# yynil/RWKV_LM_EXT

Hardware: AMD Instinct MI355X
Metric: WKV6 fwd+bwd tokens/sec/GPU (B=8,T=4096,C=2048) + %HBM roofline (higher is better)
Workload: dtype bf16

## Files before the change

### rwkv_lm_ext_amd/_build.py

```python
import os
import shutil
import subprocess

PKG_DIR = os.path.dirname(os.path.abspath(__file__))
CSRC = os.path.join(PKG_DIR, "csrc")
LIB_PATH = os.path.join(PKG_DIR, "librwkv6_amd.so")
SOURCES = ["wkv6_scan.hip", "wkv5_scan.hip", "wkv6_chunk.hip", "wkv6_chunk_bwd12k.hip", "wkv6_mix.hip", "wkv6_lora.hip", "wkv6_api.hip"]
HEADERS = ["wkv6_common.h", "wkv6_scan.h", "wkv5_scan.h", "wkv6_chunk.h", os.path.join("..", "..", "include", "wkv6_amd.h")]
HIPCC_FLAGS = ["--offload-arch=gfx950", "-O3", "-std=c++17", "-fPIC", "-fno-strict-aliasing", "-Wall", "-Wno-unused-function"]


def _hipcc():
    return shutil.which("hipcc") or "/opt/rocm/bin/hipcc"


def needs_build():
    if not os.path.exists(LIB_PATH):
        return True
    t = os.path.getmtime(LIB_PATH)
    deps = [os.path.join(CSRC, s) for s in SOURCES + HEADERS] + [os.path.abspath(__file__)]
    return any(os.path.exists(d) and os.path.getmtime(d) > t for d in deps)


def build(force=False, verbose=False):
    import fcntl
    import tempfile
    if not force and not needs_build():
        return LIB_PATH
    with open(LIB_PATH + ".lock", "w") as lock:
        fcntl.flock(lock, fcntl.LOCK_EX)
        try:
            if not force and not needs_build():
                return LIB_PATH
            with tempfile.TemporaryDirectory(prefix="rwkv6_build_", dir=PKG_DIR) as tmp:
                objs = []
                for src in SOURCES:
                    obj = os.path.join(tmp, src.replace(".hip", ".o"))
                    cmd = [_hipcc()] + HIPCC_FLAGS + ["-c", os.path.join(CSRC, src), "-o", obj]
                    if verbose:
                        print(" ".join(cmd))
                    subprocess.check_call(cmd)
                    objs.append(obj)
                out = os.path.join(tmp, "librwkv6_amd.so")
                cmd = [_hipcc(), "--offload-arch=gfx950", "-shared", "-fPIC", "-o", out] + objs
                if verbose:
                    print(" ".join(cmd))
                subprocess.check_call(cmd)
                os.replace(out, LIB_PATH)
            return LIB_PATH
        finally:
            fcntl.flock(lock, fcntl.LOCK_UN)


if __name__ == "__main__":
    print(build(force=True, verbose=True))
```

### rwkv_lm_ext_amd/csrc/wkv6_chunk_bwd12k.hip

```cpp
#include <type_traits>
#include "wkv6_chunk.h"

namespace wkv6 {

namespace {

using namespace chunk;

enum { R_RH = 0, R_RL, R_GY, R_R, R_K, NR_ARR };
enum { K_KH = 0, K_KL, K_V, NK_ARR };
constexpr int FRS = 72 * 4;
constexpr int ROFF_FR = NR_ARR * ARR;
constexpr int ROFF_LW = ROFF_FR + BLK * FRS;
constexpr int ROFF_E8 = ROFF_LW + BLK * FRS;
constexpr int ROFF_COEF = ROFF_E8 + 256;
constexpr int ROFF_VG = ROFF_COEF + 128;
constexpr int RBLK_BYTES = ROFF_VG + 128;
constexpr int KOFF_E16 = NK_ARR * ARR;
constexpr int KOFF_E16M8 = KOFF_E16 + 256;
constexpr int KBLK_BYTES = KOFF_E16M8 + 256;
constexpr int STG = 32, SBLK = STG / BLK;
constexpr int RBUF_BYTES = SBLK * RBLK_BYTES;
constexpr int KBUF_BYTES = SBLK * KBLK_BYTES;
constexpr int KRING = 3;
constexpr int KP_OFF = 2 * RBUF_BYTES;
constexpr int CKT = CKPT_TOK;
constexpr int XT_OFF = KP_OFF + KRING * KBUF_BYTES;
constexpr int XS_OFF = XT_OFF + 4 * 1024;
constexpr int XFLAG_OFF = 128;
constexpr int GRS = 144;
constexpr int GOP_OFF = XS_OFF + 2 * 1024;
constexpr int TAG_DA = 0, TAG_SC = 4, TAG_GA = 8, TAG_GB = 12, TAG_GC = 16, TAG_GD = 20, N_TAGS = 24;
constexpr int BWD12K_LDS = GOP_OFF + 2 * HEAD * GRS;
static_assert(BWD12K_LDS <= 160 * 1024, "LDS budget");

#define WKV6_DPP_ACC4(x, ctrl) asm("s_nop 1\n\t" \
    "v_add_f32_dpp %0, %0, %0 " ctrl " row_mask:0xf bank_mask:0xf\n\t" "v_add_f32_dpp %1, %1, %1 " ctrl " row_mask:0xf bank_mask:0xf\n\t" \
    "v_add_f32_dpp %2, %2, %2 " ctrl " row_mask:0xf bank_mask:0xf\n\t" "v_add_f32_dpp %3, %3, %3 " ctrl " row_mask:0xf bank_mask:0xf" \
    : "+v"(x[0]), "+v"(x[1]), "+v"(x[2]), "+v"(x[3]))

__device__ __forceinline__ void split8(const float (&t0)[4], const float (&t1)[4], b8v& hi, b8v& lo, const SplitConst& spc)
{
    uint2 h0, l0, h1, l1;
    split4(t0, h0, l0, spc);
    split4(t1, h1, l1, spc);
    hi = __builtin_bit_cast(b8v, make_uint4(h0.x, h0.y, h1.x, h1.y));
    lo = __builtin_bit_cast(b8v, make_uint4(l0.x, l0.y, l1.x, l1.y));
}

enum : unsigned {
    BWD_W_RAW = 1u << 0,
    BWD_SPLIT = 1u << 1,
    BWD_AFF = 1u << 2,
    BWD_CLK = 1u << 3,
    BWD_CHAIN = 1u << 4,
    BWD_VARLEN = 1u << 5,
};
constexpr unsigned bit(bool on, unsigned b) { return on ? b : 0u; }
struct BwdChain {
    int b, ntok;
    int ko, ro;
    bool chained_in;
    bool nx_chain;
    unsigned nx_bh;
    int nx_b, nx_ntok;
    bool nx_rev, nx_use_u;
    const float* nx_ckpt;
};
struct BwdCarry {
    uint2 pr[2], pk[2], pw[2];
    float4 pe[2];
    uint2 ck_[2];
    float cfr[2][4], clw[2][4], cc8[4];
    uint2 cvp[2];
    f4v CK[4];
};
template <unsigned MODE, int GEN = 0, int ROLE = 0>
__device__ __forceinline__ void chunk_bwd12k_body(const ScanArgs& a, const unsigned slot, BwdCarry& cy, const unsigned sslot = 0, const BwdChain& ch = BwdChain{})
{
    constexpr bool W_RAW = (MODE & BWD_W_RAW) != 0;
    constexpr bool SPLIT = (MODE & BWD_SPLIT) != 0;
    constexpr bool AFF = (MODE & BWD_AFF) != 0;
    constexpr bool CLK = (MODE & BWD_CLK) != 0;
    constexpr bool CHAIN = (MODE & BWD_CHAIN) != 0;
    constexpr bool VARLEN = (MODE & BWD_VARLEN) != 0;
    [[maybe_unused]] const bool chained_in = CHAIN && ch.chained_in, nx_chain = CHAIN && ch.nx_chain;
    [[maybe_unused]] const int ko = CHAIN ? ch.ko : 0, ro = CHAIN ? ch.ro : 0;
    extern __shared__ __attribute__((aligned(16))) char smem[];
    int tid_ = threadIdx.x;
    if constexpr (CHAIN) asm volatile("" : "+v"(tid_));
    const int tid = tid_, lane = tid & 63;
    const SplitConst spc = split_const();
    const int hwid = __builtin_amdgcn_readfirstlane(tid >> 6);
    const int part = SPLIT ? (int)(slot & 1) : 0;
    const int bh = SPLIT ? (int)(slot >> 1) : (int)slot;
    const int wid = SPLIT ? (hwid < 4 ? hwid + 4 * part : hwid + 4) : hwid;
    const bool rowrole = ROLE ? ROLE == 1 : wid < 4, producer = ROLE ? ROLE == 3 : wid >= 8;
    const int wv = wid & 3;
    const int pb = wid & 1, half = (wid >> 1) & 1;
    const int b = CHAIN ? ch.b : (a.order ? a.order[bh / a.H] : bh / a.H), h = bh % a.H;
    const long base = VARLEN ? (long)a.tok_off[b] * a.C + (long)h * HEAD : (long)b * a.T * a.C + (long)h * HEAD;
    const bf16_t* const gr_ = reinterpret_cast<const bf16_t*>(a.r) + base;
    const bf16_t* const gk_ = reinterpret_cast<const bf16_t*>(a.k) + base;
    const bf16_t* const gv_ = reinterpret_cast<const bf16_t*>(a.v) + base;
    const bf16_t* const ggy = reinterpret_cast<const bf16_t*>(a.gy) + base;
    bf16_t* const ogr = reinterpret_cast<bf16_t*>(a.gr) + base;
    bf16_t* const ogk = reinterpret_cast<bf16_t*>(a.gk) + base;
    bf16_t* const ogv = reinterpret_cast<bf16_t*>(a.gv) + base;
    bf16_t* const ogw = reinterpret_cast<bf16_t*>(a.gw) + base;
    int ntok = a.T;
    if constexpr (CHAIN) ntok = ch.ntok;
    else if (a.lens) ntok = min(max(a.lens[b], 0), a.T);
    const TokAddr<AFF> tok(a, b, ntok);
    const int C_ = a.C;
    const unsigned nbytes = ntok > 0 ? (unsigned)(ntok - 1) * a.C * 2u + 128u : 0u;
    const rsrc_t rs_gr = make_rsrc(ogr, nbytes), rs_gk = make_rsrc(ogk, nbytes), rs_gv = make_rsrc(ogv, nbytes), rs_gw = make_rsrc(ogw, nbytes);
    const long sbase = (GEN && a.side_compact) ? (long)sslot * a.T * HEAD : base;
    const unsigned sstr = (GEN && a.side_compact) ? (unsigned)HEAD : (unsigned)a.C;
    const unsigned nbytes4 = ntok > 0 ? (unsigned)(ntok - 1) * sstr * 4u + 256u : 0u;
    const rsrc_t rs_side[4] = {make_rsrc(GEN && a.g_f32[0] ? a.g_f32[0] + sbase : nullptr, GEN && a.g_f32[0] ? nbytes4 : 0u),
                               make_rsrc(GEN && a.g_f32[1] ? a.g_f32[1] + sbase : nullptr, GEN && a.g_f32[1] ? nbytes4 : 0u),
                               make_rsrc(GEN && a.g_f32[2] ? a.g_f32[2] + sbase : nullptr, GEN && a.g_f32[2] ? nbytes4 : 0u),
                               make_rsrc(GEN && a.g_f32[3] ? a.g_f32[3] + sbase : nullptr, GEN && a.g_f32[3] ? nbytes4 : 0u)};
    const int lp_side = tok.lane(lane & 15, 16 * wv + 4 * (lane >> 4), (int)sstr);
    const int lp_put = tok.lane((((lane >> 4) & 1) ? 0 : BLK) + (lane & 15), 16 * wv + 8 * (lane >> 5), C_);
    auto fetch_old = [&](int which, const rsrc_t& rs, int pu, unsigned bit, float (&old)[4]) {
        if constexpr (GEN == 2) {
            const unsigned idx = tok.off(pu, lane & 15, 16 * wv + 4 * (lane >> 4), (int)sstr, bit, lp_side);
            const float4 t = buf_load16f(rs_side[which], idx * 4u);
            old[0] = t.x; old[1] = t.y; old[2] = t.z; old[3] = t.w;
        }
    };
#ifdef WKV6_STAMP
    unsigned long long stamp_acc[6] = {0, 0, 0, 0, 0, 0}, ts0 = 0, ts1 = 0, ts2 = 0, ts3 = 0, ts4 = 0, ts5 = 0;
    unsigned long long tp0 = 0, tp1 = 0;
    unsigned long long poll_acc[8] = {0, 0, 0, 0, 0, 0, 0, 0};
#define WKV6_ACCP(idx, t1, t0) do { stamp_acc[5] += (t1) - (t0); poll_acc[(idx) >> 2] += (t1) - (t0); } while (0)
#else
#define WKV6_ACCP(idx, t1, t0) do { } while (0)
#endif
    const int x_ = lane & 15, g_ = lane >> 4;
    typedef unsigned v2u_t __attribute__((ext_vector_type(2)));
    typedef unsigned v4u_t __attribute__((ext_vector_type(4)));
    typedef volatile v4u_t __attribute__((address_space(3))) lds_vv4u;
    [[maybe_unused]] uint2 held_st[4] = {};
    auto put = [&](int which, const rsrc_t& rs, int stg, int blk, unsigned bit, uint2 v) {
        if constexpr (GEN == 1) return;
        if (blk == SBLK - 1) { held_st[which] = v; return; }
        const auto sx = __builtin_amdgcn_permlane16_swap(held_st[which].x, v.x, false, false);
        const auto sy = __builtin_amdgcn_permlane16_swap(held_st[which].y, v.y, false, false);
        buf_store16(rs, tok.off(stg * STG, ((g_ & 1) ? 0 : BLK) + x_, 16 * wv + 8 * (g_ >> 1), C_, bit, lp_put) * 2u,
                    make_uint4(sx[0], sy[0], sx[1], sy[1]));
    };
    auto emit = [&](int which, int stg, int blk, unsigned bit, float (&o)[4], const float (&old)[4]) -> uint2 {
        if constexpr (GEN == 1) {
            const unsigned idx = tok.off(stg * STG + blk * BLK, x_, 16 * wv + 4 * g_, (int)sstr, bit, lp_side);
            buf_store16f(rs_side[which], idx * 4u, o);
            return make_uint2(0u, 0u);
        }
        if constexpr (GEN == 2) {
#pragma unroll
            for (int q = 0; q < 4; ++q) o[q] += old[q];
        }
        return make_uint2(pack_bf2(o[0], o[1]), pack_bf2(o[2], o[3]));
    };

#ifdef WKV6_DEBUGBUF
    unsigned long long clk0 = 0, rtc0 = 0, clk1 = 0, rtc1 = 0;
    WKV6_CLK(clk0, rtc0);
#endif
    if constexpr (CLK) { if (hwid == 0) clock_stamp(a, slot, 0); }
    const int ngrp = (ntok + STG - 1) / STG;
    auto rpart = [&](int stg, int blk) { return smem + ((stg + ro) & 1) * RBUF_BYTES + blk * RBLK_BYTES; };
    auto kpart = [&](int stg, int blk) { return smem + KP_OFF + (int)((unsigned)(stg + ko) % (unsigned)KRING) * KBUF_BYTES + blk * KBLK_BYTES; };
    [[maybe_unused]] auto rpart_nx = [&](int e, int blk) { return smem + ((ro + 1 + e) & 1) * RBUF_BYTES + blk * RBLK_BYTES; };
    [[maybe_unused]] auto kpart_nx = [&](int e, int blk) { return smem + KP_OFF + (int)((unsigned)(ko + 2 * KRING - 1 - e) % (unsigned)KRING) * KBUF_BYTES + blk * KBLK_BYTES; };

    const int c8i = lane & 7, tq = lane >> 3;
    const int ch0 = 32 * half + 4 * c8i;
    float uu[4] = {0.f, 0.f, 0.f, 0.f};
    if (a.use_u) io4<bf16_t>::load(reinterpret_cast<const bf16_t*>(a.u) + h * HEAD + ch0, uu);

    uint2 (&pr)[2] = cy.pr, (&pk)[2] = cy.pk, (&pw)[2] = cy.pw;
    float4 (&pe)[2] = cy.pe;
    uint2 (&ck_)[2] = cy.ck_;
    uint2 pv[2], pg[2], cv_[2];
    float (&cfr)[2][4] = cy.cfr, (&clw)[2][4] = cy.clw, (&cc8)[4] = cy.cc8;
    if (!chained_in) { cc8[0] = 0.f; cc8[1] = 0.f; cc8[2] = 0.f; cc8[3] = 0.f; }
    const rsrc_t rs_r = make_rsrc(gr_, nbytes), rs_k = make_rsrc(gk_, nbytes), rs_v = make_rsrc(gv_, nbytes), rs_g = make_rsrc(ggy, nbytes);
    const rsrc_t rs_w = W_RAW ? make_rsrc(reinterpret_cast<const bf16_t*>(a.w) + base, nbytes)
                              : make_rsrc(reinterpret_cast<const float*>(a.w) + base, ntok > 0 ? (unsigned)(ntok - 1) * a.C * 4u + 256u : 0u);
    struct RowIn {
        rsrc_t r, k, v, g, w;
        TokAddr<AFF> tok;
    };
    const RowIn cur{rs_r, rs_k, rs_v, rs_g, rs_w, tok};
    [[maybe_unused]] auto row_in_of = [&](int b_, int h_, int ntok_, bool rev_) {
        const long base_ = (long)b_ * a.T * a.C + (long)h_ * HEAD;
        const unsigned nb_ = ntok_ > 0 ? (unsigned)(ntok_ - 1) * a.C * 2u + 128u : 0u;
        return RowIn{make_rsrc(reinterpret_cast<const bf16_t*>(a.r) + base_, nb_), make_rsrc(reinterpret_cast<const bf16_t*>(a.k) + base_, nb_),
                     make_rsrc(reinterpret_cast<const bf16_t*>(a.v) + base_, nb_), make_rsrc(reinterpret_cast<const bf16_t*>(a.gy) + base_, nb_),
                     W_RAW ? make_rsrc(reinterpret_cast<const bf16_t*>(a.w) + base_, nb_)
                           : make_rsrc(reinterpret_cast<const float*>(a.w) + base_, ntok_ > 0 ? (unsigned)(ntok_ - 1) * a.C * 4u + 256u : 0u),
                     TokAddr<AFF>(ntok_, rev_)};
    };
    const int lp_in[2] = {tok.lane(pb * BLK + 2 * tq, ch0, C_), tok.lane(pb * BLK + 2 * tq + 1, ch0, C_)};
    auto load_r = [&](const RowIn& in, const int (&lp)[2], int stg) {
#pragma unroll
        for (int tt = 0; tt < 2; ++tt) {
            pr[tt] = buf_load8(in.r, in.tok.off(stg * STG, pb * BLK + 2 * tq + tt, ch0, C_, REV_R, lp[tt]) * 2u);
            if constexpr (SPLIT) pg[tt] = buf_load8(in.g, in.tok.off(stg * STG, pb * BLK + 2 * tq + tt, ch0, C_, REV_Y, lp[tt]) * 2u);
        }
    };
    auto load_kw = [&](const RowIn& in, const int (&lp)[2], int stg) {
#pragma unroll
        for (int tt = 0; tt < 2; ++tt) {
            const int pl = pb * BLK + 2 * tq + tt;
            const unsigned ik = in.tok.off(stg * STG, pl, ch0, C_, REV_K, lp[tt]), iw = in.tok.off(stg * STG, pl, ch0, C_, REV_W, lp[tt]);
            pk[tt] = buf_load8(in.k, ik * 2u);
            if constexpr (SPLIT) pv[tt] = buf_load8(in.v, in.tok.off(stg * STG, pl, ch0, C_, REV_V, lp[tt]) * 2u);
            if constexpr (W_RAW) pw[tt] = buf_load8(in.w, iw * 2u);
            else pe[tt] = buf_load16f(in.w, iw * 4u);
        }
    };
    auto prep = [&](auto HASR, auto HASK, char* const rb, char* const kb, int sk, int ntok_k, const float (&uu)[4],
                    const RowIn& rq, const int (&rq_lp)[2], int next_r, int next_k) {
        float r[2][4], ko[2][4], k[2][4], cs[2][4], lwn[2][4], coef[2] = {0.f, 0.f};
        if constexpr (HASR) {
#pragma unroll
            for (int tt = 0; tt < 2; ++tt) {
                r[tt][0] = bf_lo(pr[tt].x); r[tt][1] = bf_hi(pr[tt].x); r[tt][2] = bf_lo(pr[tt].y); r[tt][3] = bf_hi(pr[tt].y);
                ko[tt][0] = bf_lo(ck_[tt].x); ko[tt][1] = bf_hi(ck_[tt].x); ko[tt][2] = bf_lo(ck_[tt].y); ko[tt][3] = bf_hi(ck_[tt].y);
                float part = 0.f;
#pragma unroll
                for (int c = 0; c < 4; ++c) part = fmaf(r[tt][c] * uu[c], ko[tt][c], part);
                part += dpp_mov<DPP_XOR1>(part);
                part += dpp_mov<DPP_XOR2>(part);
                part += dpp_mov<DPP_SHL4>(part);
                coef[tt] = part;
                const int tok = 2 * tq + tt;
                char* const rowz = rb + tok * RSB + ((ch0 * 2) ^ ((tok & 8) << 1));
                *reinterpret_cast<uint2*>(rowz + R_R * ARR) = pr[tt];
                *reinterpret_cast<uint2*>(rowz + R_K * ARR) = ck_[tt];
                *reinterpret_cast<float4*>(rb + ROFF_LW + tok * FRS + ch0 * 4) = make_float4(clw[tt][0], clw[tt][1], clw[tt][2], clw[tt][3]);
                if constexpr (SPLIT) {
                    *reinterpret_cast<uint2*>(rb + tok * RSB + ch0 * 2 + R_GY * ARR) = pg[tt];
                    typedef __bf16 bf2 __attribute__((ext_vector_type(2)));
                    float pvg = __builtin_amdgcn_fdot2_f32_bf16(__builtin_bit_cast(bf2, pg[tt].x), __builtin_bit_cast(bf2, cv_[tt].x), 0.f, false);
                    pvg = __builtin_amdgcn_fdot2_f32_bf16(__builtin_bit_cast(bf2, pg[tt].y), __builtin_bit_cast(bf2, cv_[tt].y), pvg, false);
                    pvg += dpp_mov<DPP_XOR1>(pvg);
                    pvg += dpp_mov<DPP_XOR2>(pvg);
                    pvg += dpp_mov<DPP_SHL4>(pvg);
                    if (c8i == 0) *reinterpret_cast<float*>(rb + ROFF_VG + (half * 16 + tok) * 4) = pvg;
                }
            }
        }
        if constexpr (HASR) load_r(rq, rq_lp, next_r);
        if constexpr (HASK) {
#pragma unroll
            for (int tt = 0; tt < 2; ++tt) {
                const bool valid = sk * STG + pb * BLK + 2 * tq + tt < ntok_k;
                k[tt][0] = bf_lo(pk[tt].x); k[tt][1] = bf_hi(pk[tt].x); k[tt][2] = bf_lo(pk[tt].y); k[tt][3] = bf_hi(pk[tt].y);
                ck_[tt] = pk[tt];
                if constexpr (SPLIT) {
                    *reinterpret_cast<uint2*>(kb + (2 * tq + tt) * RSB + ch0 * 2 + K_V * ARR) = pv[tt];
                    cv_[tt] = pv[tt];
                }
                float lw[4];
                if constexpr (W_RAW) {
                    lw[0] = -exp2_fast(LOG2E * bf_lo(pw[tt].x)); lw[1] = -exp2_fast(LOG2E * bf_hi(pw[tt].x));
                    lw[2] = -exp2_fast(LOG2E * bf_lo(pw[tt].y)); lw[3] = -exp2_fast(LOG2E * bf_hi(pw[tt].y));
                } else {
                    lw[0] = pe[tt].x; lw[1] = pe[tt].y; lw[2] = pe[tt].z; lw[3] = pe[tt].w;
                }
#pragma unroll
                for (int c = 0; c < 4; ++c) {
                    const float l = valid ? fmaxf(lw[c] * LOG2E, LW_MIN2) : 0.f;
                    cs[tt][c] = tt ? cs[tt - 1][c] + l : l;
                    lwn[tt][c] = valid ? lw[c] : 0.f;
                }
            }
            if (__builtin_amdgcn_ballot_w64(lwn[0][0] < LW_MIN || lwn[0][1] < LW_MIN || lwn[0][2] < LW_MIN || lwn[0][3] < LW_MIN ||
                                            lwn[1][0] < LW_MIN || lwn[1][1] < LW_MIN || lwn[1][2] < LW_MIN || lwn[1][3] < LW_MIN)) {
#pragma unroll
                for (int tt = 0; tt < 2; ++tt)
#pragma unroll
                    for (int c = 0; c < 4; ++c) lwn[tt][c] *= exp2_fast(LOG2E * fminf(lwn[tt][c] - LW_MIN, 0.f));
            }
            load_kw(rq, rq_lp, next_k);
        } else {
#pragma unroll
            for (int tt = 0; tt < 2; ++tt)
#pragma unroll
                for (int c = 0; c < 4; ++c) { k[tt][c] = 0.f; cs[tt][c] = 0.f; lwn[tt][c] = 0.f; }
        }
        float pre[4], c8[4], c16[4];
#pragma unroll
        for (int c = 0; c < 4; ++c) {
            float tot = cs[1][c], a_, b_;
            const float t = dpp_mov<DPP_ROR8>(tot);
            float pfx = (tq & 1) ? t : 0.f;
            tot += t;
            rows16(tot, a_, b_);
            pfx += (tq & 2) ? a_ : 0.f;
            tot = a_ + b_;
            halves32(tot, a_, b_);
            pfx += (tq & 4) ? a_ : 0.f;
            pre[c] = pfx;
            c8[c] = a_;
            c16[c] = a_ + b_;
        }
        if constexpr (HASR) {
#pragma unroll
            for (int tt = 0; tt < 2; ++tt) {
                float rh[4], fr[4];
#pragma unroll
                for (int c = 0; c < 4; ++c) {
                    fr[c] = exp2_fast(cfr[tt][c]);
                    rh[c] = r[tt][c] * fr[c];
                }
                const int tok = 2 * tq + tt;
                char* const row = rb + tok * RSB + ch0 * 2;
                uint2 hi, lo;
                split4(rh, hi, lo, spc);
                *reinterpret_cast<uint2*>(row + R_RH * ARR) = hi; *reinterpret_cast<uint2*>(row + R_RL * ARR) = lo;
                *reinterpret_cast<float4*>(rb + ROFF_FR + tok * FRS + ch0 * 4) = make_float4(fr[0], fr[1], fr[2], fr[3]);
            }
        }
#pragma unroll
        for (int tt = 0; tt < 2; ++tt) {
            float kh[4];
#pragma unroll
            for (int c = 0; c < 4; ++c) {
                const float cex = tt ? pre[c] + cs[tt - 1][c] : pre[c];
                const float cin = pre[c] + cs[tt][c];
                cfr[tt][c] = cex - c8[c];
                clw[tt][c] = lwn[tt][c];
                kh[c] = k[tt][c] * exp2_fast(c8[c] - cin);
            }
            if constexpr (HASK) {
                char* const row = kb + (2 * tq + tt) * RSB + ch0 * 2;
                uint2 hi, lo;
                split4(kh, hi, lo, spc);
                *reinterpret_cast<uint2*>(row + K_KH * ARR) = hi; *reinterpret_cast<uint2*>(row + K_KL * ARR) = lo;
            }
        }
        if constexpr (HASR) {
            if (c8i == 0) {
                *reinterpret_cast<float*>(rb + ROFF_COEF + (half * 16 + 2 * tq) * 4) = coef[0];
                *reinterpret_cast<float*>(rb + ROFF_COEF + (half * 16 + 2 * tq + 1) * 4) = coef[1];
            }
        }
        if (tq == 0) {
            if constexpr (HASR)
                *reinterpret_cast<float4*>(rb + ROFF_E8 + ch0 * 4) =
                    make_float4(exp2_fast(cc8[0]), exp2_fast(cc8[1]), exp2_fast(cc8[2]), exp2_fast(cc8[3]));
            if constexpr (HASK) {
                *reinterpret_cast<float4*>(kb + KOFF_E16 + ch0 * 4) =
                    make_float4(exp2_fast(c16[0]), exp2_fast(c16[1]), exp2_fast(c16[2]), exp2_fast(c16[3]));
                *reinterpret_cast<float4*>(kb + KOFF_E16M8 + ch0 * 4) =
                    make_float4(exp2_fast(c16[0] - c8[0]), exp2_fast(c16[1] - c8[1]), exp2_fast(c16[2] - c8[2]), exp2_fast(c16[3] - c8[3]));
            }
        }
#pragma unroll
        for (int c = 0; c < 4; ++c) cc8[c] = c8[c];
    };

    const int x = lane & 15, g = lane >> 4;
    int troff = (4 * g + (x >> 2)) * RSB + 8 * (x & 3);
    int trow = (4 * g + (x >> 2)) * RSB + 16 * (x & 3);
    auto cat2 = [](s4v a_, s4v b_) { return __builtin_bit_cast(b8v, __builtin_shufflevector(a_, b_, 0, 1, 2, 3, 4, 5, 6, 7)); };
    typedef volatile int __attribute__((address_space(3))) lds_vint;
    auto xflag_at = [&](int idx) { return (lds_vint*)(smem + (idx >> 3) * RSB + XFLAG_OFF + (idx & 7) * 4); };
    if (tid < N_TAGS) *xflag_at(tid) = 0;
    unsigned tag_wv = (unsigned)(unsigned long)(lds_vint*)(smem + XFLAG_OFF + 4 * wv);
    unsigned tag_tb = (unsigned)(unsigned long)(lds_vint*)(smem + XFLAG_OFF + 8 * (wv & 1));
    asm volatile("" : "+v"(tag_wv), "+v"(tag_tb));
    auto tag_off = [](int idx0) { return (idx0 >> 3) * RSB + (idx0 & 7) * 4; };
    auto publish_at = [&](unsigned base, int idx0, int extra, int tagv) {
        if (lane == 0) *(lds_vint*)(unsigned long)(base + (unsigned)(tag_off(idx0) + extra)) = tagv;
    };
    auto publish = [&](int idx0, int tagv) { publish_at(tag_wv, idx0, 0, tagv); };
#ifdef WKV6_DEBUG
    auto spin_fail = [&](int idx, int tag, unsigned seen) {
        if (a.aux && lane == 0) {
            unsigned* const d = reinterpret_cast<unsigned*>(a.aux);
            d[0] = 0xdeadbeefu; d[1] = slot; d[2] = (unsigned)((wid << 8) | idx); d[3] = (unsigned)tag; d[4] = seen;
        }
        __builtin_trap();
    };
#define WKV6_SPIN_GUARD(idx, tag, seen) if (++spins > (1u << 22)) spin_fail(idx, tag, seen)
#else
#define WKV6_SPIN_GUARD(idx, tag, seen) do { } while (0)
#endif
    const int lane_tag4 = (lane & 3) * 4, lane_tag2 = (lane & 1) * 4;
    auto tags_differ = [&](unsigned f, int tag) { return __builtin_amdgcn_ballot_w64(f != (unsigned)tag) != 0; };
    auto await_n = [&](int idx, int tag, int lane_off) {
        [[maybe_unused]] unsigned spins = 0;
        WKV6_T(tp0);
        for (;;) {
            const unsigned f = (unsigned)*(lds_vint*)((unsigned char __attribute__((address_space(3)))*)xflag_at(idx) + lane_off);
            if (!tags_differ(f, tag)) break;
            WKV6_SPIN_GUARD(idx, tag, f);
            __builtin_amdgcn_s_sleep(1);
        }
        WKV6_T(tp1); WKV6_ACCP(idx, tp1, tp0);
    };
    auto await2 = [&](int idx, int tag) { await_n(idx, tag, lane_tag2); };
    auto await4 = [&](int idx, int tag) { await_n(idx, tag, lane_tag4); };
    auto peek4 = [&](int idx) -> unsigned {
        return (unsigned)*(lds_vint*)((unsigned char __attribute__((address_space(3)))*)xflag_at(idx) + lane_tag4);
    };
    auto settle4 = [&](int idx, int tag, const unsigned f) { if (tags_differ(f, tag)) await4(idx, tag); };
    auto tile_store = [&](int off, uint2 hi, uint2 lo) {
        *(lds_vv4u*)(smem + off + lane * 16) = v4u_t{hi.x, hi.y, lo.x, lo.y};
    };
    auto tile_load = [&](int off) {
        const v4u_t f = *(lds_vv4u*)(smem + off + lane * 16);
        return make_uint4(f.x, f.y, f.z, f.w);
    };
    constexpr std::true_type yes_c{};
    constexpr std::false_type no_c{};
    [[maybe_unused]] const int nxn = CHAIN ? (ch.nx_ntok + STG - 1) / STG : 0;
    if (producer) {
        if (!chained_in && ngrp > 0) {
            load_kw(cur, lp_in, ngrp - 1);
            load_r(cur, lp_in, ngrp - 1);
            prep(no_c, yes_c, rpart(0, pb), kpart(ngrp - 1, pb), ngrp - 1, ntok, uu, cur, lp_in, -1, ngrp - 2);
            if (ngrp > 1) prep(yes_c, yes_c, rpart(ngrp - 1, pb), kpart(ngrp - 2, pb), ngrp - 2, ntok, uu, cur, lp_in, ngrp - 2, ngrp - 3);
            else prep(yes_c, no_c, rpart(0, pb), kpart(0, pb), -1, ntok, uu, cur, lp_in, -1, -1);
        }
        __syncthreads();
        for (int grp = ngrp - 1; grp >= 2; --grp) {
            WKV6_T(ts0);
#ifdef WKV6_STAMP
            asm volatile("" :: "v"(pr[0].x), "v"(pk[0].x), "v"(pr[1].x), "v"(pk[1].x));
#endif
            WKV6_T(ts1);
            WKV6_T(ts2);
            prep(yes_c, yes_c, rpart(grp - 1, pb), kpart(grp - 2, pb), grp - 2, ntok, uu, cur, lp_in, grp - 2, grp - 3);
            WKV6_T(ts3);
            __syncthreads();
            WKV6_T(ts4);
            WKV6_ACC(0, ts1, ts0); WKV6_ACC(1, ts2, ts1); WKV6_ACC(2, ts3, ts2); WKV6_ACC(3, ts4, ts3);
        }
        bool chained_out = false;
        if constexpr (CHAIN) {
            if (nx_chain) {
                const int nxh = (int)(ch.nx_bh % (unsigned)a.H);
                const RowIn nx = row_in_of(ch.nx_b, nxh, ch.nx_ntok, ch.nx_rev);
                const int lp_nx[2] = {nx.tok.lane(pb * BLK + 2 * tq, ch0, C_), nx.tok.lane(pb * BLK + 2 * tq + 1, ch0, C_)};
                float uu_nx[4] = {0.f, 0.f, 0.f, 0.f};
                if (ch.nx_use_u) io4<bf16_t>::load(reinterpret_cast<const bf16_t*>(a.u) + nxh * HEAD + ch0, uu_nx);
                load_kw(nx, lp_nx, nxn - 1);
                prep(yes_c, yes_c, rpart(0, pb), kpart_nx(0, pb), nxn - 1, ch.nx_ntok, uu, nx, lp_nx, nxn - 1, nxn - 2);
                __syncthreads();
                prep(yes_c, yes_c, rpart_nx(0, pb), kpart_nx(1, pb), nxn - 2, ch.nx_ntok, uu_nx, nx, lp_nx, nxn - 2, nxn - 3);
                __syncthreads();
                chained_out = true;
            }
        }
        if (!chained_out) {
            if (ngrp >= 2) {
                prep(yes_c, no_c, rpart(0, pb), kpart(0, pb), -1, ntok, uu, cur, lp_in, -1, -1);
                __syncthreads();
            }
            if (ngrp >= 1) __syncthreads();
        }
    } else
    if (rowrole) {
        float ue[4] = {0.f, 0.f, 0.f, 0.f};
        if (a.use_u) io4<bf16_t>::load(reinterpret_cast<const bf16_t*>(a.u) + h * HEAD + 16 * wv + 4 * g, ue);
        f4v ST[SBLK][4], GI[4];
#pragma unroll
        for (int t = 0; t < 4; ++t) GI[t] = f4v{0.f, 0.f, 0.f, 0.f};
        float Rc[4] = {0.f, 0.f, 0.f, 0.f}, gu_acc[4] = {0.f, 0.f, 0.f, 0.f};
        if (a.rc_in) io4<float>::load(a.rc_in + (long)b * a.C + h * HEAD + 16 * wv + 4 * g, Rc);
        const unsigned nslots = VARLEN ? ((unsigned)ntok + CKT - 1) / CKT : ((unsigned)a.T + CKT - 1) / CKT;
        const int segs = a.ckpt_segs > 1 ? a.ckpt_segs : 1;
        const long ck_slot0 = VARLEN ? (long)h * a.ck_stride + a.ck_off[b] : ((long)((b / segs) * a.H + h) * segs + b % segs) * nslots;
        const rsrc_t rs_ck = make_rsrc(a.ckpt + ck_slot0 * (HEAD * HEAD), nslots * 16384u);
        f4v (&CK)[4] = cy.CK;
        auto request_ckpt = [&](int stg) {
            const unsigned off = (unsigned)(stg >> 1) * 16384u + (unsigned)wv * 4096u + (unsigned)lane * 16u;
#pragma unroll
            for (int jt = 0; jt < 4; ++jt) {
                const float4 t = buf_load16f(rs_ck, off + jt * 1024u);
                CK[jt] = f4v{t.x, t.y, t.z, t.w};
            }
        };
        auto advance = [&](const char* kb, const f4v (&Sin)[4], f4v (&Sout)[4]) {
            const s4v khf = tr_read(kb + K_KH * ARR + troff + 32 * wv);
            const s4v klf = tr_read(kb + K_KL * ARR + troff + 32 * wv);
            const float e16 = *reinterpret_cast<const float*>(kb + KOFF_E16 + (16 * wv + x) * 4);
            const float e16m8 = *reinterpret_cast<const float*>(kb + KOFF_E16M8 + (16 * wv + x) * 4);
#pragma unroll
            for (int jt = 0; jt < 4; ++jt) {
                const s4v vf = tr_read(kb + K_V * ARR + trow + tile_tr(jt));
                f4v o = {0.f, 0.f, 0.f, 0.f};
                o = mfma32(cat2(vf, vf), cat2(khf, klf), o);
#pragma unroll
                for (int q = 0; q < 4; ++q) Sout[jt][q] = fmaf(e16, Sin[jt][q], e16m8 * o[q]);
            }
        };
        if constexpr (CHAIN) { if (!chained_in && ngrp > 0) request_ckpt(ngrp - 1); }
#pragma unroll
        for (int q = 0; q < 4; ++q) asm volatile("" : "+v"(ue[q]), "+v"(Rc[q]));
        if constexpr (!CHAIN) { if (ngrp > 0) request_ckpt(ngrp - 1); }
        {
            unsigned none_bytes = 0u;
            if constexpr (CHAIN) { asm volatile("" : "+s"(none_bytes)); none_bytes = __builtin_amdgcn_readfirstlane(none_bytes); }
            const rsrc_t rs_none = make_rsrc(static_cast<bf16_t*>(nullptr), none_bytes);
#pragma unroll
            for (int i = 0; i < (GEN == 1 ? 4 : 3); ++i)
                buf_store16(rs_none, 16u * i, make_uint4(__float_as_uint(ue[0]), __float_as_uint(ue[1]), __float_as_uint(ue[2]), __float_as_uint(ue[3])));
        }

        __syncthreads();
        for (int grp = ngrp - 1; grp >= 0; --grp) {
            int tagv = grp + 1;
            asm volatile("" : "+v"(tagv));
            WKV6_T(ts0);
            f4v gvb[SBLK];
            auto take_gop = [&](int blk) {
                int base_ = GOP_OFF + (8 * g + (x >> 2)) * GRS + (16 * wv + 4 * (x & 3)) * 2;
                asm volatile("" : "+v"(base_));
                typedef short s8v __attribute__((ext_vector_type(8)));
                const char* const kb = kpart(grp, blk);
                f4v acc = {0.f, 0.f, 0.f, 0.f};
#pragma unroll
                for (int s = 0; s < 2; ++s) {
                    const char* const ph = smem + base_ + 32 * s * GRS;
                    const s8v h8 = __builtin_shufflevector(tr_read(ph), tr_read(ph + 4 * GRS), 0, 1, 2, 3, 4, 5, 6, 7);
                    const s8v l8 = __builtin_shufflevector(tr_read(ph + HEAD * GRS), tr_read(ph + HEAD * GRS + 4 * GRS), 0, 1, 2, 3, 4, 5, 6, 7);
                    const b8v vr = ld_b8(kb + K_V * ARR + x * RSB + (32 * s + 8 * g) * 2);
                    acc = mfma32(__builtin_bit_cast(b8v, h8), vr, acc);
                    acc = mfma32(__builtin_bit_cast(b8v, l8), vr, acc);
                }
                return acc;
            };
            if constexpr (!SPLIT) {
                if (grp == ngrp - 1) await4(TAG_GA, grp + 1);
                gvb[1] = take_gop(1);
                publish(TAG_GB, tagv);
            }
            float old_gr[SBLK][4] = {}, old_gk[SBLK][4] = {}, old_gw[SBLK][4] = {};
#pragma unroll
            for (int blk = SBLK - 1; blk >= 0; --blk) fetch_old(0, rs_gr, grp * STG + blk * BLK, REV_R, old_gr[blk]);
            if (wv >= 2) {
                const int tb = wv - 2;
                const char* const rb = rpart(grp, tb);
                const char* const kb = kpart(grp, tb);
                f4v dA_ab = {0.f, 0.f, 0.f, 0.f}, dA_ba = {0.f, 0.f, 0.f, 0.f};
#pragma unroll
                for (int s = 0; s < 2; ++s) {
                    const int off = x * RSB + (32 * s + 8 * g) * 2;
                    const b8v gy_ = ld_b8(rb + R_GY * ARR + off), vr = ld_b8(kb + K_V * ARR + off);
                    dA_ab = mfma32(gy_, vr, dA_ab);
                    dA_ba = mfma32(vr, gy_, dA_ba);
                }
                float dab[4], dba[4];
#pragma unroll
                for (int q = 0; q < 4; ++q) {
                    const int o = 4 * g + q;
                    dab[q] = x < o ? dA_ab[q] : 0.f;
                    dba[q] = o < x ? dA_ba[q] : 0.f;
                }
                uint2 th, tl;
                split4(dab, th, tl, spc);
                tile_store(XT_OFF + (2 * tb) * 1024, th, tl);
                publish_at(tag_tb, TAG_DA, 0, tagv);
                split4(dba, th, tl, spc);
                tile_store(XT_OFF + (2 * tb + 1) * 1024, th, tl);
                publish_at(tag_tb, TAG_DA, 4, tagv);
            } else if constexpr (!SPLIT) {
                const char* const rb = rpart(grp, wv);
                const char* const kb = kpart(grp, wv);
                f4v sc = {0.f, 0.f, 0.f, 0.f};
#pragma unroll
                for (int s = 0; s < 2; ++s) {
                    const int off = x * RSB + (32 * s + 8 * g) * 2;
                    const b8v rh = ld_b8(rb + R_RH * ARR + off), rl = ld_b8(rb + R_RL * ARR + off);
                    const b8v kh = ld_b8(kb + K_KH * ARR + off), kl = ld_b8(kb + K_KL * ARR + off);
                    sc = mfma32(rh, kh, sc);
                    sc = mfma32(rh, kl, sc);
                    sc = mfma32(rl, kh, sc);
                }
                const float4 cfa = *reinterpret_cast<const float4*>(rb + ROFF_COEF + 16 * g);
                const float4 cfb = *reinterpret_cast<const float4*>(rb + ROFF_COEF + 64 + 16 * g);
                const float cf[4] = {cfa.x + cfb.x, cfa.y + cfb.y, cfa.z + cfb.z, cfa.w + cfb.w};
                float scm[4];
#pragma unroll
                for (int q = 0; q < 4; ++q) {
                    const int o = 4 * g + q;
                    scm[q] = x < o ? sc[q] : (x == o ? cf[q] : 0.f);
                }
                uint2 th, tl;
                split4(scm, th, tl, spc);
                tile_store(XS_OFF + wv * 1024, th, tl);
                publish(TAG_SC, tagv);
            }
#pragma unroll
            for (int jt = 0; jt < 4; ++jt) ST[0][jt] = CK[jt];
            WKV6_T(ts1);
            if (grp & 1) {
                advance(kpart(grp - 1, 0), ST[0], ST[0]);
                advance(kpart(grp - 1, 1), ST[0], ST[0]);
            }
            [[maybe_unused]] unsigned pk_gc = 0;
#pragma unroll
            for (int blk = 0; blk < SBLK - 1; ++blk) advance(kpart(grp, blk), ST[blk], ST[blk + 1]);
            const unsigned pk_da = peek4(TAG_DA);
            WKV6_T(ts2);
            f4v ackp[SBLK];
            float at[SBLK][4], vgs[SBLK];
            uint2 held_gr[SBLK];
#pragma unroll
            for (int blk = SBLK - 1; blk >= 0; --blk) {
                const char* const rb = rpart(grp, blk);
                const char* const kb = kpart(grp, blk);
                b8v gyr[2];
#pragma unroll
                for (int s = 0; s < 2; ++s) gyr[s] = ld_b8(rb + R_GY * ARR + x * RSB + (32 * s + 8 * g) * 2);
                const float vg = *reinterpret_cast<const float*>(rb + ROFF_VG + x * 4) + *reinterpret_cast<const float*>(rb + ROFF_VG + 64 + x * 4);
                vgs[blk] = vg;
                if (blk == SBLK - 1) settle4(TAG_DA, grp + 1, pk_da);
                if constexpr (!SPLIT) { if (blk == 0) pk_gc = peek4(TAG_GC); }
                const uint4 fab = tile_load(XT_OFF + (2 * blk) * 1024), fba = tile_load(XT_OFF + (2 * blk + 1) * 1024);
                const s4v dab_hi = __builtin_bit_cast(s4v, make_uint2(fab.x, fab.y)), dab_lo = __builtin_bit_cast(s4v, make_uint2(fab.z, fab.w));
                const s4v dba_hi = __builtin_bit_cast(s4v, make_uint2(fba.x, fba.y)), dba_lo = __builtin_bit_cast(s4v, make_uint2(fba.z, fba.w));
                const s4v rhf_w = tr_read(rb + R_RH * ARR + troff + 32 * wv);
                const s4v rlf_w = tr_read(rb + R_RL * ARR + troff + 32 * wv);
                const s4v khf = tr_read(kb + K_KH * ARR + troff + 32 * wv);
                const s4v klf = tr_read(kb + K_KL * ARR + troff + 32 * wv);
                const float4 e8o = *reinterpret_cast<const float4*>(rb + ROFF_E8 + (16 * wv + 4 * g) * 4);
                f4v accs = {0.f, 0.f, 0.f, 0.f};
#pragma unroll
                for (int s = 0; s < 2; ++s) {
                    float t0[4], t1[4];
                    b8v hi, lo;
#pragma unroll
                    for (int q = 0; q < 4; ++q) { t0[q] = ST[blk][2 * s][q]; t1[q] = ST[blk][2 * s + 1][q]; }
                    split8(t0, t1, hi, lo, spc);
                    accs = mfma32(hi, gyr[s], accs);
                    accs = mfma32(lo, gyr[s], accs);
                }
                f4v accr16 = {0.f, 0.f, 0.f, 0.f};
                accr16 = mfma16(khf, dba_hi, accr16);
                accr16 = mfma16(khf, dba_lo, accr16);
                accr16 = mfma16(klf, dba_hi, accr16);
                const f4v accr = {fmaf(e8o.x, accs[0], accr16[0]), fmaf(e8o.y, accs[1], accr16[1]),
                                  fmaf(e8o.z, accs[2], accr16[2]), fmaf(e8o.w, accs[3], accr16[3])};
                f4v ak = {0.f, 0.f, 0.f, 0.f};
                ak = mfma16(rhf_w, dab_hi, ak);
                ak = mfma16(rhf_w, dab_lo, ak);
                ak = mfma16(rlf_w, dab_hi, ak);
                ackp[blk] = ak;
                {
                    const int ch = 16 * wv + 4 * g;
                    const float4 fr4 = *reinterpret_cast<const float4*>(rb + ROFF_FR + x * FRS + ch * 4);
                    const uint2 rr = *reinterpret_cast<const uint2*>(rb + R_R * ARR + x * RSB + ((ch * 2) ^ ((x & 8) << 1)));
                    const uint2 kk = *reinterpret_cast<const uint2*>(rb + R_K * ARR + x * RSB + ((ch * 2) ^ ((x & 8) << 1)));
                    const float frv[4] = {fr4.x, fr4.y, fr4.z, fr4.w};
                    const float rv[4] = {bf_lo(rr.x), bf_hi(rr.x), bf_lo(rr.y), bf_hi(rr.y)};
                    const float kv[4] = {bf_lo(kk.x), bf_hi(kk.x), bf_lo(kk.y), bf_hi(kk.y)};
                    float o_gr[4];
#pragma unroll
                    for (int q = 0; q < 4; ++q) {
                        const float dq = frv[q] * accr[q];
                        o_gr[q] = fmaf(vg * ue[q], kv[q], dq);
                        gu_acc[q] = fmaf(vg * rv[q], kv[q], gu_acc[q]);
                        at[blk][q] = rv[q] * dq;
                    }
                    held_gr[blk] = emit(0, grp, blk, REV_R, o_gr, old_gr[blk]);
                }
            }
            WKV6_T(ts3);
#pragma unroll
            for (int blk = SBLK - 1; blk >= 0; --blk) {
                fetch_old(1, rs_gk, grp * STG + blk * BLK, REV_K, old_gk[blk]);
                fetch_old(3, rs_gw, grp * STG + blk * BLK, REV_W, old_gw[blk]);
            }
            if (grp > 0 && !(grp & 1)) request_ckpt(grp - 1);
            if constexpr (CHAIN) {
                if (nx_chain && grp == 0) {
                    const rsrc_t rs_nx = make_rsrc(ch.nx_ckpt + ((long)ch.nx_b * a.H + (long)(ch.nx_bh % (unsigned)a.H)) * nslots * (HEAD * HEAD), nslots * 16384u);
                    const unsigned off = (unsigned)((nxn - 1) >> 1) * 16384u + (unsigned)wv * 4096u + (unsigned)lane * 16u;
#pragma unroll
                    for (int jt = 0; jt < 4; ++jt) {
                        const float4 t = buf_load16f(rs_nx, off + jt * 1024u);
                        CK[jt] = f4v{t.x, t.y, t.z, t.w};
                    }
                }
            }
            if constexpr (!SPLIT) {
                settle4(TAG_GC, grp + 1, pk_gc);
                gvb[0] = take_gop(0);
                publish(TAG_GD, tagv);
            }
#pragma unroll
            for (int blk = SBLK - 1; blk >= 0; --blk) put(0, rs_gr, grp, blk, REV_R, held_gr[blk]);
#pragma unroll
            for (int blk = SBLK - 1; blk >= 0; --blk) {
                const char* const rb = rpart(grp, blk);
                const char* const kb = kpart(grp, blk);
                f4v acck = {0.f, 0.f, 0.f, 0.f};
                [[maybe_unused]] f4v Oi[4];
                [[maybe_unused]] float e8x = 0.f, e16x = 0.f;
                if constexpr (SPLIT) {
                    e8x = *reinterpret_cast<const float*>(rb + ROFF_E8 + (16 * wv + x) * 4);
                    e16x = *reinterpret_cast<const float*>(kb + KOFF_E16 + (16 * wv + x) * 4);
                    const float e16m8x = *reinterpret_cast<const float*>(kb + KOFF_E16M8 + (16 * wv + x) * 4);
                    const s4v rhf_w = tr_read(rb + R_RH * ARR + troff + 32 * wv);
                    const s4v rlf_w = tr_read(rb + R_RL * ARR + troff + 32 * wv);
#pragma unroll
                    for (int jt = 0; jt < 4; ++jt) {
                        const s4v gyf = tr_read(rb + R_GY * ARR + trow + tile_tr(jt));
                        f4v o = {0.f, 0.f, 0.f, 0.f};
                        o = mfma32(cat2(gyf, gyf), cat2(rhf_w, rlf_w), o);
                        Oi[jt] = o;
                    }
#pragma unroll
                    for (int s = 0; s < 2; ++s) {
                        const b8v vr = ld_b8(kb + K_V * ARR + x * RSB + (32 * s + 8 * g) * 2);
                        float t0[4], t1[4];
                        b8v hi, lo;
#pragma unroll
                        for (int q = 0; q < 4; ++q) { t0[q] = GI[2 * s][q] * e16m8x; t1[q] = GI[2 * s + 1][q] * e16m8x; }
                        split8(t0, t1, hi, lo, spc);
                        acck = mfma32(hi, vr, acck);
                        acck = mfma32(lo, vr, acck);
                    }
                } else {
                    acck = gvb[blk];
                }
                acck += ackp[blk];
                {
                    const int ch = 16 * wv + 4 * g;
                    const float4 fn4 = *reinterpret_cast<const float4*>(x < 15 ? rb + ROFF_FR + (x + 1) * FRS + ch * 4 : kb + KOFF_E16M8 + ch * 4);
                    const float4 fk4 = make_float4(__builtin_amdgcn_rcpf(fn4.x), __builtin_amdgcn_rcpf(fn4.y), __builtin_amdgcn_rcpf(fn4.z),
                                                   __builtin_amdgcn_rcpf(fn4.w));
                    const float4 lw4 = *reinterpret_cast<const float4*>(rb + ROFF_LW + x * FRS + ch * 4);
                    const uint2 rr = *reinterpret_cast<const uint2*>(rb + R_R * ARR + x * RSB + ((ch * 2) ^ ((x & 8) << 1)));
                    const uint2 kk = *reinterpret_cast<const uint2*>(rb + R_K * ARR + x * RSB + ((ch * 2) ^ ((x & 8) << 1)));
                    const float fkv[4] = {fk4.x, fk4.y, fk4.z, fk4.w}, lwv[4] = {lw4.x, lw4.y, lw4.z, lw4.w};
                    const float rv[4] = {bf_lo(rr.x), bf_hi(rr.x), bf_lo(rr.y), bf_hi(rr.y)};
                    const float kv[4] = {bf_lo(kk.x), bf_hi(kk.x), bf_lo(kk.y), bf_hi(kk.y)};
                    const float vg = vgs[blk];
                    float o_gk[4], o_gw[4], bt[4], dl[4], sfx[4];
#pragma unroll
                    for (int q = 0; q < 4; ++q) {
                        const float dk = fkv[q] * acck[q];
                        o_gk[q] = fmaf(vg * ue[q], rv[q], dk);
                        bt[q] = kv[q] * dk;
                        dl[q] = at[blk][q] - bt[q];
                        sfx[q] = dl[q];
                    }
                    WKV6_DPP_ACC4(sfx, "row_shl:1");
                    WKV6_DPP_ACC4(sfx, "row_shl:2");
                    WKV6_DPP_ACC4(sfx, "row_shl:4");
                    WKV6_DPP_ACC4(sfx, "row_shl:8");
#pragma unroll
                    for (int q = 0; q < 4; ++q) {
                        const float total = dpp_mov<DPP_BCAST0>(sfx[q]);
                        o_gw[q] = (Rc[q] + (sfx[q] - dl[q]) - bt[q]) * lwv[q];
                        Rc[q] += total;
                    }
                    put(1, rs_gk, grp, blk, REV_K, emit(1, grp, blk, REV_K, o_gk, old_gk[blk]));
                    put(3, rs_gw, grp, blk, REV_W, emit(3, grp, blk, REV_W, o_gw, old_gw[blk]));
                }
                if constexpr (SPLIT) {
#pragma unroll
                    for (int jt = 0; jt < 4; ++jt)
#pragma unroll
                        for (int q = 0; q < 4; ++q) GI[jt][q] = fmaf(e16x, GI[jt][q], e8x * Oi[jt][q]);
                }
            }
            WKV6_T(ts4);
            __syncthreads();
            WKV6_T(ts5);
            WKV6_ACC(0, ts1, ts0); WKV6_ACC(1, ts2, ts1); WKV6_ACC(2, ts3, ts2); WKV6_ACC(3, ts4, ts3); WKV6_ACC(4, ts5, ts4);
        }
        if (a.gu) {
            float s4[4];
#pragma unroll
            for (int q = 0; q < 4; ++q) s4[q] = row_sum16(gu_acc[q]);
            const long o = (long)b * a.C + h * HEAD + 16 * wv + 4 * g;
            if (x == 0) {
                if (a.part_f32) io4<float>::store(reinterpret_cast<float*>(a.gu) + o, s4);
                else io4<bf16_t>::store(reinterpret_cast<bf16_t*>(a.gu) + o, s4);
            }
        }
    } else {
        f4v GJ[4];
#pragma unroll
        for (int t = 0; t < 4; ++t) {
            float t4[4] = {0.f, 0.f, 0.f, 0.f};
            if (a.g_in)
                io4<float>::load(a.g_in + ((long)b * a.H + h) * HEAD * HEAD + (long)(16 * wv + x) * HEAD + tile_ch(t) + 8 * g, t4);
            GJ[t] = f4v{t4[0], t4[1], t4[2], t4[3]};
        }
#pragma unroll
        for (int t = 0; t < 4; ++t) asm volatile("" : "+v"(GJ[t]));
        const int tl = lane >> 4, cl = lane & 15;
        uint2 cv[SBLK], cg[SBLK];
        uint2 (&cvp)[SBLK] = cy.cvp;
        const int lp_vg = tok.lane(4 * wv + tl, 4 * cl, C_);
        auto load_v = [&](const RowIn& in, int lp, int stg) {
#pragma unroll
            for (int blk = 0; blk < SBLK; ++blk) {
                cv[blk] = buf_load8(in.v, in.tok.off(stg * STG + blk * BLK, 4 * wv + tl, 4 * cl, C_, REV_V, lp) * 2u);
            }
        };
        auto load_gy = [&](const RowIn& in, int lp, int stg) {
#pragma unroll
            for (int blk = 0; blk < SBLK; ++blk) {
                cg[blk] = buf_load8(in.g, in.tok.off(stg * STG + blk * BLK, 4 * wv + tl, 4 * cl, C_, REV_Y, lp) * 2u);
            }
        };
        auto copy_v = [&](char* const k0) {
#pragma unroll
            for (int blk = 0; blk < SBLK; ++blk) {
                *reinterpret_cast<uint2*>(k0 + blk * KBLK_BYTES + K_V * ARR + (4 * wv + tl) * RSB + 8 * cl) = cv[blk];
                cvp[blk] = cv[blk];
            }
        };
        auto copy_gy = [&](char* const r0) {
#pragma unroll
            for (int blk = 0; blk < SBLK; ++blk) {
                char* const rb = r0 + blk * RBLK_BYTES;
                const int tok = 4 * wv + tl;
                *reinterpret_cast<uint2*>(rb + R_GY * ARR + tok * RSB + 8 * cl) = cg[blk];
                typedef __bf16 bf2 __attribute__((ext_vector_type(2)));
                float vg = __builtin_amdgcn_fdot2_f32_bf16(__builtin_bit_cast(bf2, cg[blk].x), __builtin_bit_cast(bf2, cvp[blk].x), 0.f, false);
                vg = __builtin_amdgcn_fdot2_f32_bf16(__builtin_bit_cast(bf2, cg[blk].y), __builtin_bit_cast(bf2, cvp[blk].y), vg, false);
                vg += dpp_mov<DPP_XOR1>(vg);
                vg += dpp_mov<DPP_XOR2>(vg);
                vg += dpp_mov<DPP_SHL4>(vg);
                if ((cl & 7) == 0) *reinterpret_cast<float*>(rb + ROFF_VG + ((cl >> 3) * 16 + tok) * 4) = vg;
            }
        };
        [[maybe_unused]] RowIn nx = cur;
        [[maybe_unused]] int lp_vg_nx = lp_vg;
        if constexpr (CHAIN) {
            if (nx_chain) {
                nx = row_in_of(ch.nx_b, (int)(ch.nx_bh % (unsigned)a.H), ch.nx_ntok, ch.nx_rev);
                lp_vg_nx = nx.tok.lane(4 * wv + tl, 4 * cl, C_);
            }
        }
        auto scale_split = [&](const char* kb, b8v (&h)[2], b8v (&l)[2]) {
#pragma unroll
            for (int s = 0; s < 2; ++s) {
                float t0[4], t1[4];
                const float4 m0 = *reinterpret_cast<const float4*>(kb + KOFF_E16M8 + (32 * s + 8 * g) * 4);
                const float4 m1 = *reinterpret_cast<const float4*>(kb + KOFF_E16M8 + (32 * s + 8 * g + 4) * 4);
                t0[0] = GJ[2 * s][0] * m0.x; t0[1] = GJ[2 * s][1] * m0.y; t0[2] = GJ[2 * s][2] * m0.z; t0[3] = GJ[2 * s][3] * m0.w;
                t1[0] = GJ[2 * s + 1][0] * m1.x; t1[1] = GJ[2 * s + 1][1] * m1.y;
                t1[2] = GJ[2 * s + 1][2] * m1.z; t1[3] = GJ[2 * s + 1][3] * m1.w;
                split8(t0, t1, h[s], l[s], spc);
            }
        };
        auto gop_write = [&](const b8v (&h)[2], const b8v (&l)[2]) {
#pragma unroll
            for (int s = 0; s < 2; ++s) {
                char* const dst = smem + GOP_OFF + (16 * wv + x) * GRS + (32 * s + 8 * g) * 2;
                *(lds_vv4u*)dst = __builtin_bit_cast(v4u_t, h[s]);
                *(lds_vv4u*)(dst + HEAD * GRS) = __builtin_bit_cast(v4u_t, l[s]);
            }
        };
        [[maybe_unused]] b8v nh[2] = {}, nl[2] = {};
        if (!SPLIT && !chained_in && ngrp > 0) {
            load_v(cur, lp_vg, ngrp - 1);
            load_gy(cur, lp_vg, ngrp - 1);
            copy_v(kpart(ngrp - 1, 0));
            copy_gy(rpart(ngrp - 1, 0));
            if (ngrp > 1) {
                load_v(cur, lp_vg, ngrp - 2);
                copy_v(kpart(ngrp - 2, 0));
            }
        }
        __syncthreads();
        if constexpr (!SPLIT) { if (ngrp > 0) scale_split(kpart(ngrp - 1, SBLK - 1), nh, nl); }
        for (int grp = ngrp - 1; grp >= 0; --grp) {
            int tagv = grp + 1;
            for (int i_ = 0; i_ < wv; ++i_) __builtin_amdgcn_s_sleep(2);
            asm volatile("" : "+v"(tagv));
            WKV6_T(ts0);

            s4v gyT_w[SBLK], sc_hi[SBLK], sc_lo[SBLK];
            f4v accp[SBLK];
            b8v gh[SBLK][2], gl[SBLK][2];
            [[maybe_unused]] f4v Og[SBLK][4];
            if constexpr (!SPLIT)
#pragma unroll
            for (int blk = SBLK - 1; blk >= 0; --blk) {
                const char* const rb = rpart(grp, blk);
                const char* const kb = kpart(grp, blk);
                if (blk == SBLK - 1) {
#pragma unroll
                    for (int s = 0; s < 2; ++s) { gh[blk][s] = nh[s]; gl[blk][s] = nl[s]; }
                    if (grp == ngrp - 1) {
                        gop_write(gh[blk], gl[blk]);
                        publish(TAG_GA, tagv);
                    }
                    if constexpr (CHAIN) {
                        const bool g_nx = nx_chain && grp == 0, v_nx = nx_chain && grp <= 1;
                        load_gy(g_nx ? nx : cur, g_nx ? lp_vg_nx : lp_vg, g_nx ? nxn - 1 : grp - 1);
                        load_v(v_nx ? nx : cur, v_nx ? lp_vg_nx : lp_vg, v_nx ? (grp == 1 ? nxn - 1 : nxn - 2) : grp - 2);
                    } else {
                        if (grp > 0) load_gy(cur, lp_vg, grp - 1);
                        if (grp > 1) load_v(cur, lp_vg, grp - 2);
                    }
                } else {
                    scale_split(kb, gh[blk], gl[blk]);
                    await4(TAG_GB, grp + 1);
                    gop_write(gh[blk], gl[blk]);
                    publish(TAG_GC, tagv);
                }
                const s4v gyT = tr_read(rb + R_GY * ARR + troff + 32 * wv);
#pragma unroll
                for (int it = 0; it < 4; ++it) {
                    const s4v rhf = tr_read(rb + R_RH * ARR + trow + tile_tr(it));
                    const s4v rlf = tr_read(rb + R_RL * ARR + trow + tile_tr(it));
                    f4v o = {0.f, 0.f, 0.f, 0.f};
                    o = mfma32(cat2(rhf, rlf), cat2(gyT, gyT), o);
                    const float4 d16 = *reinterpret_cast<const float4*>(kb + KOFF_E16 + (tile_ch(it) + 8 * g) * 4);
                    const float4 d8 = *reinterpret_cast<const float4*>(rb + ROFF_E8 + (tile_ch(it) + 8 * g) * 4);
                    GJ[it][0] = fmaf(d16.x, GJ[it][0], d8.x * o[0]);
                    GJ[it][1] = fmaf(d16.y, GJ[it][1], d8.y * o[1]);
                    GJ[it][2] = fmaf(d16.z, GJ[it][2], d8.z * o[2]);
                    GJ[it][3] = fmaf(d16.w, GJ[it][3], d8.w * o[3]);
                }
            }
            float old_gv[SBLK][4] = {};
#pragma unroll
            for (int blk = SBLK - 1; blk >= 0; --blk) fetch_old(2, rs_gv, grp * STG + blk * BLK, REV_V, old_gv[blk]);
            if (SPLIT && wv < SBLK) {
                const char* const rb = rpart(grp, wv);
                const char* const kb = kpart(grp, wv);
                f4v sc = {0.f, 0.f, 0.f, 0.f};
#pragma unroll
                for (int s = 0; s < 2; ++s) {
                    const int off = x * RSB + (32 * s + 8 * g) * 2;
                    const b8v rh = ld_b8(rb + R_RH * ARR + off), rl = ld_b8(rb + R_RL * ARR + off);
                    const b8v kh = ld_b8(kb + K_KH * ARR + off), kl = ld_b8(kb + K_KL * ARR + off);
                    sc = mfma32(rh, kh, sc);
                    sc = mfma32(rh, kl, sc);
                    sc = mfma32(rl, kh, sc);
                }
                const float4 cfa = *reinterpret_cast<const float4*>(rb + ROFF_COEF + 16 * g);
                const float4 cfb = *reinterpret_cast<const float4*>(rb + ROFF_COEF + 64 + 16 * g);
                const float cf[4] = {cfa.x + cfb.x, cfa.y + cfb.y, cfa.z + cfb.z, cfa.w + cfb.w};
                float scm[4];
#pragma unroll
                for (int q = 0; q < 4; ++q) {
                    const int o = 4 * g + q;
                    scm[q] = x < o ? sc[q] : (x == o ? cf[q] : 0.f);
                }
                uint2 th, tl;
                split4(scm, th, tl, spc);
                tile_store(XS_OFF + wv * 1024, th, tl);
                publish(TAG_SC, tagv);
            }
#pragma unroll
            for (int blk = 0; blk < SBLK; ++blk) gyT_w[blk] = tr_read(rpart(grp, blk) + R_GY * ARR + troff + 32 * wv);
#pragma unroll
            for (int blk = 0; blk < SBLK; ++blk) {
                if (blk == 0) await2(TAG_SC, grp + 1);
                const uint4 f = tile_load(XS_OFF + blk * 1024);
                sc_hi[blk] = __builtin_bit_cast(s4v, make_uint2(f.x, f.y));
                sc_lo[blk] = __builtin_bit_cast(s4v, make_uint2(f.z, f.w));
            }
#pragma unroll
            for (int blk = 0; blk < SBLK; ++blk) {
                f4v acc = {0.f, 0.f, 0.f, 0.f};
                acc = mfma32(cat2(gyT_w[blk], gyT_w[blk]), cat2(sc_hi[blk], sc_lo[blk]), acc);
                accp[blk] = acc;
                if constexpr (SPLIT) {
                    const char* const rb = rpart(grp, blk);
#pragma unroll
                    for (int it = 0; it < 4; ++it) {
                        const s4v rhf = tr_read(rb + R_RH * ARR + trow + tile_tr(it));
                        const s4v rlf = tr_read(rb + R_RL * ARR + trow + tile_tr(it));
                        f4v o = {0.f, 0.f, 0.f, 0.f};
                        o = mfma32(cat2(rhf, rlf), cat2(gyT_w[blk], gyT_w[blk]), o);
                        Og[blk][it] = o;
                    }
                }
            }
            WKV6_T(ts1);
            uint2 held_gv[SBLK];
#pragma unroll
            for (int blk = SBLK - 1; blk >= 0; --blk) {
                const char* const kb = kpart(grp, blk);
                f4v acc = {0.f, 0.f, 0.f, 0.f};
#pragma unroll
                for (int s = 0; s < 2; ++s) {
                    const int off = x * RSB + (32 * s + 8 * g) * 2;
                    const b8v kh = ld_b8(kb + K_KH * ARR + off), kl = ld_b8(kb + K_KL * ARR + off);
                    if constexpr (SPLIT) {
                        float t0[4], t1[4];
                        const float4 m0 = *reinterpret_cast<const float4*>(kb + KOFF_E16M8 + (32 * s + 8 * g) * 4);
                        const float4 m1 = *reinterpret_cast<const float4*>(kb + KOFF_E16M8 + (32 * s + 8 * g + 4) * 4);
                        t0[0] = GJ[2 * s][0] * m0.x; t0[1] = GJ[2 * s][1] * m0.y; t0[2] = GJ[2 * s][2] * m0.z; t0[3] = GJ[2 * s][3] * m0.w;
                        t1[0] = GJ[2 * s + 1][0] * m1.x; t1[1] = GJ[2 * s + 1][1] * m1.y;
                        t1[2] = GJ[2 * s + 1][2] * m1.z; t1[3] = GJ[2 * s + 1][3] * m1.w;
                        split8(t0, t1, gh[blk][s], gl[blk][s], spc);
                    }
                    acc = mfma32(gh[blk][s], kh, acc);
                    acc = mfma32(gh[blk][s], kl, acc);
                    acc = mfma32(gl[blk][s], kh, acc);
                }
                acc += accp[blk];
                {
                    float o[4] = {acc[0], acc[1], acc[2], acc[3]};
                    held_gv[blk] = emit(2, grp, blk, REV_V, o, old_gv[blk]);
                }
                if constexpr (SPLIT) {
                    const char* const rb = rpart(grp, blk);
#pragma unroll
                    for (int it = 0; it < 4; ++it) {
                        const float4 d16 = *reinterpret_cast<const float4*>(kb + KOFF_E16 + (tile_ch(it) + 8 * g) * 4);
                        const float4 d8 = *reinterpret_cast<const float4*>(rb + ROFF_E8 + (tile_ch(it) + 8 * g) * 4);
                        GJ[it][0] = fmaf(d16.x, GJ[it][0], d8.x * Og[blk][it][0]);
                        GJ[it][1] = fmaf(d16.y, GJ[it][1], d8.y * Og[blk][it][1]);
                        GJ[it][2] = fmaf(d16.z, GJ[it][2], d8.z * Og[blk][it][2]);
                        GJ[it][3] = fmaf(d16.w, GJ[it][3], d8.w * Og[blk][it][3]);
                    }
                }
            }
#pragma unroll
            for (int blk = SBLK - 1; blk >= 0; --blk) put(2, rs_gv, grp, blk, REV_V, held_gv[blk]);
            if constexpr (!SPLIT) {
                if (grp > 0) {
                    scale_split(kpart(grp - 1, SBLK - 1), nh, nl);
                    await4(TAG_GD, grp + 1);
                    gop_write(nh, nl);
                    publish(TAG_GA, tagv - 1);
                }
            }
            if constexpr (!SPLIT) {
                if (grp > 0) copy_gy(rpart(grp - 1, 0));
                else if (CHAIN && nx_chain) copy_gy(rpart_nx(0, 0));
                if (grp > 1) copy_v(kpart(grp - 2, 0));
                else if (CHAIN && nx_chain) copy_v(grp == 1 ? kpart_nx(0, 0) : kpart_nx(1, 0));
            }
            WKV6_T(ts2);
            __syncthreads();
            WKV6_T(ts3);
            WKV6_ACC(0, ts1, ts0); WKV6_ACC(1, ts2, ts1); WKV6_ACC(2, ts3, ts2);
        }
        if (a.gs) {
            const long so_ = ((long)b * a.H + h) * HEAD * HEAD + (long)(16 * wv + x) * HEAD + 8 * g;
#pragma unroll
            for (int it = 0; it < 4; ++it) {
                const float t4[4] = {GJ[it][0], GJ[it][1], GJ[it][2], GJ[it][3]};
                if (a.part_f32) io4<float>::store(reinterpret_cast<float*>(a.gs) + so_ + tile_ch(it), t4);
                else io4<bf16_t>::store(reinterpret_cast<bf16_t*>(a.gs) + so_ + tile_ch(it), t4);
            }
        }
    }
#ifdef WKV6_DEBUGBUF
    WKV6_CLK(clk1, rtc1);
    if (a.aux && lane == 0) {
        unsigned long long* const d = reinterpret_cast<unsigned long long*>(a.aux) + ((long)bh * 16 + wid) * 8;
#ifdef WKV6_STAMP
        for (int i = 0; i < 6; ++i) d[i] = stamp_acc[i];
        if (wid == 0 || wid == 4) for (int i = 0; i < 8; ++i) d[(12 + (wid >> 2) - wid) * 8 + i] = poll_acc[i];
#endif
        d[6] = clk1 - clk0;
        d[7] = rtc1 - rtc0;
    }
#endif
    if constexpr (CLK) { if (hwid == 0) clock_stamp(a, slot, 1); }
    if (GEN == 1 && a.zero_tail && part == 0) {
        const float z[4] = {0.f, 0.f, 0.f, 0.f};
        for (int t = ntok + (tid >> 4); t < a.T; t += (int)(blockDim.x >> 4)) {
            const unsigned idx = (unsigned)(t * a.C + 4 * (tid & 15));
            io4<bf16_t>::store(ogr + idx, z);
            io4<bf16_t>::store(ogk + idx, z);
            io4<bf16_t>::store(ogv + idx, z);
            io4<bf16_t>::store(ogw + idx, z);
        }
    }
}

template <bool W_RAW, int GEN, bool SPLIT, bool AFF>
__global__ __launch_bounds__(SPLIT ? 512 : 768) void chunk_bwd12k_kernel(const ScanArgs a)
{
    BwdCarry cy;
    chunk_bwd12k_body<bit(W_RAW, BWD_W_RAW) | bit(SPLIT, BWD_SPLIT) | bit(AFF, BWD_AFF) | bit(GEN == 0, BWD_CLK), GEN>(a, blockIdx.x, cy);
}

template <bool W_RAW>
__global__ __launch_bounds__(768) void chunk_bwd12k_varlen_kernel(const ScanArgs a)
{
    BwdCarry cy;
    chunk_bwd12k_body<bit(W_RAW, BWD_W_RAW) | BWD_AFF | BWD_VARLEN>(a, blockIdx.x, cy);
}

template <bool W_RAW>
__global__ __launch_bounds__(768) void chunk_bwd12k_varlen_rev_kernel(const ScanArgs a)
{
    BwdCarry cy;
    chunk_bwd12k_body<bit(W_RAW, BWD_W_RAW) | BWD_VARLEN>(a, blockIdx.x, cy);
}

template <bool W_RAW>
__global__ __launch_bounds__(768) void chunk_bwd12k_varlen_pair_kernel(const ScanArgs a0, const ScanArgs a1)
{
    const unsigned n = (unsigned)(a0.B * a0.H);
    const bool second = blockIdx.x >= n;
    BwdCarry cy;
    chunk_bwd12k_body<bit(W_RAW, BWD_W_RAW) | BWD_VARLEN>(second ? a1 : a0, second ? blockIdx.x - n : blockIdx.x, cy);
}

template <bool W_RAW>
__global__ __launch_bounds__(768) void chunk_bwd12k_pair_kernel(const ScanArgs a0, const ScanArgs a1)
{
    const unsigned n = (unsigned)(a0.B * a0.H);
    const bool second = blockIdx.x >= n;
    BwdCarry cy;
    chunk_bwd12k_body<bit(W_RAW, BWD_W_RAW)>(second ? a1 : a0, second ? blockIdx.x - n : blockIdx.x, cy);
}

template <bool W_RAW>
__global__ __launch_bounds__(768) void chunk_bwd12k_bi_kernel(const ScanArgs a1_, float* const ckpt2)
{
    const unsigned n = (unsigned)(a1_.B * a1_.H);
    const int H_ = a1_.H, T_ = a1_.T;
    const int* const order_ = a1_.order;
    const int* const lens_ = a1_.lens;
    const auto row_of = [&](unsigned it) { return it * gridDim.x + ((it & 1) ? gridDim.x - 1 - blockIdx.x : blockIdx.x); };
    const auto lookup = [&](unsigned row, int& b, int& ntok) {
        b = 0; ntok = 0;
        if (row < n) {
            b = order_ ? order_[row / H_] : (int)(row / H_);
            ntok = lens_ ? min(max(lens_[b], 0), T_) : T_;
        }
    };
    const int use_u_ = a1_.use_u;
    const float* const ckpt1_ = a1_.ckpt;
    const auto rows = [&](auto role_c) {
        constexpr int ROLE = decltype(role_c)::value;
        int b_cur, ntok_cur;
        lookup(row_of(0), b_cur, ntok_cur);
        BwdCarry cy;
        int ko = 0, ro = 0;
        bool chained = false;
        const auto mod3 = [](int x) { return ((x % KRING) + KRING) % KRING; };
        for (unsigned it = 0; it * gridDim.x < n; ++it) {
            const unsigned row = row_of(it);
            if (row >= n) continue;
            const unsigned row_nx = row_of(it + 1);
            int b_nx, ntok_nx;
            lookup(row_nx, b_nx, ntok_nx);
            const int n_cur = (ntok_cur + STG - 1) / STG, n_nx = (ntok_nx + STG - 1) / STG;
            const bool chain12 = n_cur >= 2, chain2n = row_nx < n && n_cur >= 2 && n_nx >= 2;
            {
                ScanArgs a1;
                load_kernargs(a1);
                chunk_bwd12k_body<bit(W_RAW, BWD_W_RAW) | BWD_AFF | BWD_CHAIN, 1, ROLE>(a1, row, cy, blockIdx.x,
                                                                                       BwdChain{b_cur, ntok_cur, ko, ro, chained, chain12, row, b_cur, ntok_cur, true, false, ckpt2});
            }
            ko = mod3(ko - n_cur); ro = (ro - n_cur) & 1;
            if constexpr (ROLE != 3) __builtin_amdgcn_fence(__ATOMIC_RELEASE, "workgroup");
            __syncthreads();
            if constexpr (ROLE != 3) __builtin_amdgcn_fence(__ATOMIC_ACQUIRE, "workgroup");
            {
                ScanArgs a2;
                load_kernargs(a2);
                a2.reverse = 1; a2.use_u = 0; a2.accumulate = 1; a2.zero_tail = 0; a2.gu = nullptr; a2.ckpt = ckpt2;
                chunk_bwd12k_body<bit(W_RAW, BWD_W_RAW) | BWD_AFF | BWD_CHAIN, 2, ROLE>(a2, row, cy, blockIdx.x,
                                                                                       BwdChain{b_cur, ntok_cur, ko, ro, chain12, chain2n, row_nx, b_nx, ntok_nx, false, use_u_ != 0, ckpt1_});
            }
            ko = mod3(ko - n_nx); ro = (ro - n_nx) & 1;
            chained = chain2n;
            __syncthreads();
            b_cur = b_nx; ntok_cur = ntok_nx;
        }
    };
    const int hw = __builtin_amdgcn_readfirstlane((int)(threadIdx.x >> 6));
    if (hw < 4) rows(std::integral_constant<int, 1>{});
    else if (hw < 8) rows(std::integral_constant<int, 2>{});
    else rows(std::integral_constant<int, 3>{});
}

template <bool W_RAW, int GEN, bool AFF> hipError_t launch_bwd12k_inst2(const ScanArgs& a, hipStream_t st)
{
    return a.split ? launch<chunk_bwd12k_kernel<W_RAW, GEN, true, AFF>>(dim3(2 * a.B * a.H), dim3(512), BWD12K_LDS, st, a)
                   : launch<chunk_bwd12k_kernel<W_RAW, GEN, false, AFF>>(dim3(a.B * a.H), dim3(768), BWD12K_LDS, st, a);
}
template <bool W_RAW, int GEN> hipError_t launch_bwd12k_inst(const ScanArgs& a, hipStream_t st)
{
    if constexpr (GEN == 0) { if (a.rev_n) return launch_bwd12k_inst2<W_RAW, 0, false>(a, st); }
    else if (a.rev_n) return hipErrorNotSupported;
    return launch_bwd12k_inst2<W_RAW, GEN, true>(a, st);
}
template <bool W_RAW> hipError_t launch_bwd12k_variant(const ScanArgs& a, hipStream_t st)
{
    const bool side = a.g_f32[0] && a.g_f32[1] && a.g_f32[2] && a.g_f32[3];
    if (a.accumulate) return side ? launch_bwd12k_inst<W_RAW, 2>(a, st) : hipErrorInvalidValue;
    const bool first_half = a.zero_tail || a.g_f32[0] || a.g_f32[1] || a.g_f32[2] || a.g_f32[3];
    if (first_half && !side) return hipErrorInvalidValue;
    return first_half ? launch_bwd12k_inst<W_RAW, 1>(a, st) : launch_bwd12k_inst<W_RAW, 0>(a, st);
}

}

hipError_t launch_chunk_state_pass(const ScanArgs& a, hipStream_t st);

hipError_t launch_chunk_bwd12k(const ScanArgs& a_, hipStream_t st)
{
    if (!a_.ckpt) return hipErrorInvalidValue;
    if (a_.split && (a_.g_in || a_.rc_in)) return hipErrorInvalidValue;
    ScanArgs a = a_;
    a.clk = clock_claim(1, &a.clk_slots);
    attach_debug_buffer(a);
    return a.wkind ? launch_bwd12k_variant<true>(a, st) : launch_bwd12k_variant<false>(a, st);
}

hipError_t launch_chunk_bwd(const ScanArgs& a_, hipStream_t st)
{
    ScanArgs a = a_;
    a.split = want_split(a.B * a.H);
    if (!offsets_fit(a)) return hipErrorInvalidValue;
    if (!a.ckpt_valid) {
        ScanArgs sp = a;
        sp.y = nullptr; sp.y_f32 = nullptr; sp.s_out = nullptr; sp.accumulate = 0; sp.zero_tail = 0;
        if (hipError_t e = launch_chunk_state_pass(sp, st)) return e;
    }
    return launch_chunk_bwd12k(a, st);
}

template <bool W_RAW> static hipError_t launch_bwd12k_varlen_inst(const ScanArgs& a, hipStream_t st)
{
    const dim3 grid(a.B * a.H);
    return a.rev_n ? launch<chunk_bwd12k_varlen_rev_kernel<W_RAW>>(grid, dim3(768), BWD12K_LDS, st, a)
                   : launch<chunk_bwd12k_varlen_kernel<W_RAW>>(grid, dim3(768), BWD12K_LDS, st, a);
}
static bool varlen_bwd_plain(const ScanArgs& a)
{
    return !(a.reverse || a.accumulate || a.zero_tail || a.g_f32[0] || a.g_f32[1] || a.g_f32[2] || a.g_f32[3] || a.g_in || a.rc_in || a.ckpt_segs > 1 ||
             a.side_compact);
}
hipError_t launch_chunk_bwd_varlen(const ScanArgs& a_, hipStream_t st)
{
    if (!a_.ckpt || !packed_arrays_ok(a_) || !offsets_fit(a_)) return hipErrorInvalidValue;
    if (!varlen_bwd_plain(a_)) return hipErrorNotSupported;
    const ScanArgs a = packed_launch_args(a_);
    if (!a.ckpt_valid) {
        ScanArgs sp = a;
        sp.y = nullptr; sp.s_out = nullptr;
        if (hipError_t e = launch_chunk_fwd_varlen(sp, true, st)) return e;
    }
    return a.wkind ? launch_bwd12k_varlen_inst<true>(a, st) : launch_bwd12k_varlen_inst<false>(a, st);
}

hipError_t launch_chunk_bwd_varlen_pair(const ScanArgs& a0_, const ScanArgs& a1_, hipStream_t st)
{
    if (!same_problem(a0_, a1_) || !packed_arrays_ok(a0_) || !same_packed_arrays(a0_, a1_) || !offsets_fit(a0_)) return hipErrorInvalidValue;
    const auto plain = [](const ScanArgs& a) { return varlen_bwd_plain(a) && a.ckpt && a.ckpt_valid; };
    if (!plain(a0_) || !plain(a1_)) return hipErrorNotSupported;
    const ScanArgs a0 = packed_launch_args(a0_), a1 = packed_launch_args(a1_);
    const dim3 grid(2 * a0.B * a0.H);
    return a0.wkind == 1 ? launch<chunk_bwd12k_varlen_pair_kernel<true>>(grid, dim3(768), BWD12K_LDS, st, a0, a1)
                         : launch<chunk_bwd12k_varlen_pair_kernel<false>>(grid, dim3(768), BWD12K_LDS, st, a0, a1);
}

hipError_t launch_chunk_bwd_bi(const ScanArgs& a1_, const ScanArgs& a2_, int* slots, hipStream_t st)
{
    const int n = bi_slots(a1_.B * a1_.H);
    if (slots) *slots = n;
    if (!n || !a1_.ckpt || !a2_.ckpt || a1_.g_in || a1_.rc_in) return hipErrorNotSupported;
    if (!offsets_fit(a1_)) return hipErrorInvalidValue;
    ScanArgs a1 = a1_, a2 = a2_;
    for (ScanArgs* a : {&a1, &a2}) {
        a->split = 0;
        if (!a->ckpt_valid) {
            ScanArgs sp = *a;
            sp.y = nullptr; sp.y_f32 = nullptr; sp.s_out = nullptr; sp.accumulate = 0; sp.zero_tail = 0;
            if (hipError_t e = launch_chunk_state_pass(sp, st)) return e;
        }
        a->side_compact = 1;
        attach_debug_buffer(*a);
    }
    return a1.wkind == 1 ? launch<chunk_bwd12k_bi_kernel<true>>(dim3(n), dim3(768), BWD12K_LDS, st, a1, a2.ckpt)
                         : launch<chunk_bwd12k_bi_kernel<false>>(dim3(n), dim3(768), BWD12K_LDS, st, a1, a2.ckpt);
}

hipError_t launch_chunk_bwd_pair(const ScanArgs& a0_, const ScanArgs& a1_, hipStream_t st)
{
    if (!same_problem(a0_, a1_)) return hipErrorInvalidValue;
    const auto plain = [](const ScanArgs& a) {
        return !a.accumulate && !a.zero_tail && !a.g_f32[0] && !a.g_f32[1] && !a.g_f32[2] && !a.g_f32[3] && a.ckpt && a.ckpt_valid;
    };
    if (!plain(a0_) || !plain(a1_)) return hipErrorNotSupported;
    if (want_split(a0_.B * a0_.H)) {
        if (hipError_t e = launch_chunk_bwd(a0_, st)) return e;
        return launch_chunk_bwd(a1_, st);
    }
    if (!offsets_fit(a0_)) return hipErrorInvalidValue;
    ScanArgs a0 = a0_, a1 = a1_;
    a0.split = a1.split = 0;
    attach_debug_buffer(a0);
    attach_debug_buffer(a1);
    const dim3 grid(2 * a0.B * a0.H);
    return a0.wkind == 1 ? launch<chunk_bwd12k_pair_kernel<true>>(grid, dim3(768), BWD12K_LDS, st, a0, a1)
                         : launch<chunk_bwd12k_pair_kernel<false>>(grid, dim3(768), BWD12K_LDS, st, a0, a1);
}

}
```

Baseline: 57.50 million.

## Unroll backward stage loops by parity to resolve LDS ring buffers at compile time

The producer and row/column stage loops of the WKV6 backward kernel are unrolled in pairs, with a compile-time parity template parameter. This lets the double-buffered R-part shared-memory address and the checkpoint-request condition resolve statically instead of through per-iteration modulo arithmetic. The stage bodies move into included files, and the u load is moved into the producer path. The cost is larger code size, more instruction-cache pressure and possible register pressure changes.

```diff
diff --git a/rwkv_lm_ext_amd/_build.py b/rwkv_lm_ext_amd/_build.py
--- a/rwkv_lm_ext_amd/_build.py
+++ b/rwkv_lm_ext_amd/_build.py
@@ -6,7 +6,8 @@
 CSRC = os.path.join(PKG_DIR, "csrc")
 LIB_PATH = os.path.join(PKG_DIR, "librwkv6_amd.so")
 SOURCES = ["wkv6_scan.hip", "wkv5_scan.hip", "wkv6_chunk.hip", "wkv6_chunk_bwd12k.hip", "wkv6_mix.hip", "wkv6_lora.hip", "wkv6_api.hip"]
-HEADERS = ["wkv6_common.h", "wkv6_scan.h", "wkv5_scan.h", "wkv6_chunk.h", os.path.join("..", "..", "include", "wkv6_amd.h")]
+HEADERS = ["wkv6_common.h", "wkv6_scan.h", "wkv5_scan.h", "wkv6_chunk.h", "wkv6_chunk_bwd12k_row_stage.inc", "wkv6_chunk_bwd12k_col_stage.inc",
+           os.path.join("..", "..", "include", "wkv6_amd.h")]
 HIPCC_FLAGS = ["--offload-arch=gfx950", "-O3", "-std=c++17", "-fPIC", "-fno-strict-aliasing", "-Wall", "-Wno-unused-function"]
 
 
diff --git a/rwkv_lm_ext_amd/csrc/wkv6_chunk_bwd12k.hip b/rwkv_lm_ext_amd/csrc/wkv6_chunk_bwd12k.hip
--- a/rwkv_lm_ext_amd/csrc/wkv6_chunk_bwd12k.hip
+++ b/rwkv_lm_ext_amd/csrc/wkv6_chunk_bwd12k.hip
@@ -57,6 +57,9 @@
     BWD_VARLEN = 1u << 5,
 };
 constexpr unsigned bit(bool on, unsigned b) { return on ? b : 0u; }
+enum { PAR_EVEN = 0, PAR_ODD = 1, PAR_RUNTIME = 2 };
+template <int P> using par_t = std::integral_constant<int, P>;
+template <int P> using par_other_t = par_t<P == PAR_RUNTIME ? PAR_RUNTIME : 1 - P>;
 struct BwdChain {
     int b, ntok;
     int ko, ro;
@@ -84,6 +87,7 @@
     constexpr bool CLK = (MODE & BWD_CLK) != 0;
     constexpr bool CHAIN = (MODE & BWD_CHAIN) != 0;
     constexpr bool VARLEN = (MODE & BWD_VARLEN) != 0;
+    constexpr bool PAIR_WALK = !CHAIN && !(GEN == 2 && !SPLIT) && !(CLK && !AFF && !SPLIT);
     [[maybe_unused]] const bool chained_in = CHAIN && ch.chained_in, nx_chain = CHAIN && ch.nx_chain;
     [[maybe_unused]] const int ko = CHAIN ? ch.ko : 0, ro = CHAIN ? ch.ro : 0;
     extern __shared__ __attribute__((aligned(16))) char smem[];
@@ -172,6 +176,15 @@
     if constexpr (CLK) { if (hwid == 0) clock_stamp(a, slot, 0); }
     const int ngrp = (ntok + STG - 1) / STG;
     auto rpart = [&](int stg, int blk) { return smem + ((stg + ro) & 1) * RBUF_BYTES + blk * RBLK_BYTES; };
+    constexpr bool R1_HOIST = SPLIT || (AFF && !VARLEN && GEN < 2);
+    [[maybe_unused]] int rbuf1 = RBUF_BYTES;
+    if constexpr (PAIR_WALK) asm("" : "+s"(rbuf1));
+    auto rpart_p = [&](auto par_c, int stg, int blk) {
+        constexpr int P = decltype(par_c)::value;
+        if constexpr (P == PAR_RUNTIME) return rpart(stg, blk);
+        else if constexpr (P == PAR_ODD) return smem + rbuf1 + blk * RBLK_BYTES;
+        else return smem + blk * RBLK_BYTES;
+    };
     auto kpart = [&](int stg, int blk) { return smem + KP_OFF + (int)((unsigned)(stg + ko) % (unsigned)KRING) * KBUF_BYTES + blk * KBLK_BYTES; };
     [[maybe_unused]] auto rpart_nx = [&](int e, int blk) { return smem + ((ro + 1 + e) & 1) * RBUF_BYTES + blk * RBLK_BYTES; };
     [[maybe_unused]] auto kpart_nx = [&](int e, int blk) { return smem + KP_OFF + (int)((unsigned)(ko + 2 * KRING - 1 - e) % (unsigned)KRING) * KBUF_BYTES + blk * KBLK_BYTES; };
@@ -179,7 +192,7 @@
     const int c8i = lane & 7, tq = lane >> 3;
     const int ch0 = 32 * half + 4 * c8i;
     float uu[4] = {0.f, 0.f, 0.f, 0.f};
-    if (a.use_u) io4<bf16_t>::load(reinterpret_cast<const bf16_t*>(a.u) + h * HEAD + ch0, uu);
+    if constexpr (!PAIR_WALK) { if (a.use_u) io4<bf16_t>::load(reinterpret_cast<const bf16_t*>(a.u) + h * HEAD + ch0, uu); }
 
     uint2 (&pr)[2] = cy.pr, (&pk)[2] = cy.pk, (&pw)[2] = cy.pw;
     float4 (&pe)[2] = cy.pe;
@@ -423,6 +436,7 @@
     constexpr std::false_type no_c{};
     [[maybe_unused]] const int nxn = CHAIN ? (ch.nx_ntok + STG - 1) / STG : 0;
     if (producer) {
+        if constexpr (PAIR_WALK) { if (a.use_u) io4<bf16_t>::load(reinterpret_cast<const bf16_t*>(a.u) + h * HEAD + ch0, uu); }
         if (!chained_in && ngrp > 0) {
             load_kw(cur, lp_in, ngrp - 1);
             load_r(cur, lp_in, ngrp - 1);
@@ -431,18 +445,34 @@
             else prep(yes_c, no_c, rpart(0, pb), kpart(0, pb), -1, ntok, uu, cur, lp_in, -1, -1);
         }
         __syncthreads();
-        for (int grp = ngrp - 1; grp >= 2; --grp) {
+        auto stage = [&](char* const rb, const int grp) { prep(yes_c, yes_c, rb, kpart(grp - 2, pb), grp - 2, ntok, uu, cur, lp_in, grp - 2, grp - 3); };
+        auto stage_head = [&]() __attribute__((always_inline)) {
             WKV6_T(ts0);
 #ifdef WKV6_STAMP
             asm volatile("" :: "v"(pr[0].x), "v"(pk[0].x), "v"(pr[1].x), "v"(pk[1].x));
 #endif
             WKV6_T(ts1);
             WKV6_T(ts2);
-            prep(yes_c, yes_c, rpart(grp - 1, pb), kpart(grp - 2, pb), grp - 2, ntok, uu, cur, lp_in, grp - 2, grp - 3);
+        };
+        auto stage_barrier = [&]() __attribute__((always_inline)) {
             WKV6_T(ts3);
             __syncthreads();
             WKV6_T(ts4);
             WKV6_ACC(0, ts1, ts0); WKV6_ACC(1, ts2, ts1); WKV6_ACC(2, ts3, ts2); WKV6_ACC(3, ts4, ts3);
+        };
+        if constexpr (!PAIR_WALK) {
+            for (int grp = ngrp - 1; grp >= 2; --grp) {
+                stage_head();
+                prep(yes_c, yes_c, rpart(grp - 1, pb), kpart(grp - 2, pb), grp - 2, ntok, uu, cur, lp_in, grp - 2, grp - 3);
+                stage_barrier();
+            }
+        } else {
+            int grp = ngrp - 1;
+            if (grp >= 2 && !(grp & 1)) { stage_head(); stage(rpart_p(par_t<PAR_ODD>{}, grp - 1, pb), grp); stage_barrier(); --grp; }
+            for (; grp >= 3; grp -= 2) {
+                stage_head(); stage(rpart_p(par_t<PAR_EVEN>{}, grp - 1, pb), grp); stage_barrier();
+                stage_head(); stage(rpart_p(par_t<PAR_ODD>{}, grp - 2, pb), grp - 1); stage_barrier();
+            }
         }
         bool chained_out = false;
         if constexpr (CHAIN) {
@@ -517,275 +547,36 @@
         }
 
         __syncthreads();
-        for (int grp = ngrp - 1; grp >= 0; --grp) {
-            int tagv = grp + 1;
-            asm volatile("" : "+v"(tagv));
-            WKV6_T(ts0);
-            f4v gvb[SBLK];
-            auto take_gop = [&](int blk) {
-                int base_ = GOP_OFF + (8 * g + (x >> 2)) * GRS + (16 * wv + 4 * (x & 3)) * 2;
-                asm volatile("" : "+v"(base_));
-                typedef short s8v __attribute__((ext_vector_type(8)));
-                const char* const kb = kpart(grp, blk);
-                f4v acc = {0.f, 0.f, 0.f, 0.f};
-#pragma unroll
-                for (int s = 0; s < 2; ++s) {
-                    const char* const ph = smem + base_ + 32 * s * GRS;
-                    const s8v h8 = __builtin_shufflevector(tr_read(ph), tr_read(ph + 4 * GRS), 0, 1, 2, 3, 4, 5, 6, 7);
-                    const s8v l8 = __builtin_shufflevector(tr_read(ph + HEAD * GRS), tr_read(ph + HEAD * GRS + 4 * GRS), 0, 1, 2, 3, 4, 5, 6, 7);
-                    const b8v vr = ld_b8(kb + K_V * ARR + x * RSB + (32 * s + 8 * g) * 2);
-                    acc = mfma32(__builtin_bit_cast(b8v, h8), vr, acc);
-                    acc = mfma32(__builtin_bit_cast(b8v, l8), vr, acc);
-                }
-                return acc;
-            };
-            if constexpr (!SPLIT) {
-                if (grp == ngrp - 1) await4(TAG_GA, grp + 1);
-                gvb[1] = take_gop(1);
-                publish(TAG_GB, tagv);
-            }
-            float old_gr[SBLK][4] = {}, old_gk[SBLK][4] = {}, old_gw[SBLK][4] = {};
-#pragma unroll
-            for (int blk = SBLK - 1; blk >= 0; --blk) fetch_old(0, rs_gr, grp * STG + blk * BLK, REV_R, old_gr[blk]);
-            if (wv >= 2) {
-                const int tb = wv - 2;
-                const char* const rb = rpart(grp, tb);
-                const char* const kb = kpart(grp, tb);
-                f4v dA_ab = {0.f, 0.f, 0.f, 0.f}, dA_ba = {0.f, 0.f, 0.f, 0.f};
-#pragma unroll
-                for (int s = 0; s < 2; ++s) {
-                    const int off = x * RSB + (32 * s + 8 * g) * 2;
-                    const b8v gy_ = ld_b8(rb + R_GY * ARR + off), vr = ld_b8(kb + K_V * ARR + off);
-                    dA_ab = mfma32(gy_, vr, dA_ab);
-                    dA_ba = mfma32(vr, gy_, dA_ba);
-                }
-                float dab[4], dba[4];
-#pragma unroll
-                for (int q = 0; q < 4; ++q) {
-                    const int o = 4 * g + q;
-                    dab[q] = x < o ? dA_ab[q] : 0.f;
-                    dba[q] = o < x ? dA_ba[q] : 0.f;
-                }
-                uint2 th, tl;
-                split4(dab, th, tl, spc);
-                tile_store(XT_OFF + (2 * tb) * 1024, th, tl);
-                publish_at(tag_tb, TAG_DA, 0, tagv);
-                split4(dba, th, tl, spc);
-                tile_store(XT_OFF + (2 * tb + 1) * 1024, th, tl);
-                publish_at(tag_tb, TAG_DA, 4, tagv);
-            } else if constexpr (!SPLIT) {
-                const char* const rb = rpart(grp, wv);
-                const char* const kb = kpart(grp, wv);
-                f4v sc = {0.f, 0.f, 0.f, 0.f};
-#pragma unroll
-                for (int s = 0; s < 2; ++s) {
-                    const int off = x * RSB + (32 * s + 8 * g) * 2;
-                    const b8v rh = ld_b8(rb + R_RH * ARR + off), rl = ld_b8(rb + R_RL * ARR + off);
-                    const b8v kh = ld_b8(kb + K_KH * ARR + off), kl = ld_b8(kb + K_KL * ARR + off);
-                    sc = mfma32(rh, kh, sc);
-                    sc = mfma32(rh, kl, sc);
-                    sc = mfma32(rl, kh, sc);
-                }
-                const float4 cfa = *reinterpret_cast<const float4*>(rb + ROFF_COEF + 16 * g);
-                const float4 cfb = *reinterpret_cast<const float4*>(rb + ROFF_COEF + 64 + 16 * g);
-                const float cf[4] = {cfa.x + cfb.x, cfa.y + cfb.y, cfa.z + cfb.z, cfa.w + cfb.w};
-                float scm[4];
-#pragma unroll
-                for (int q = 0; q < 4; ++q) {
-                    const int o = 4 * g + q;
-                    scm[q] = x < o ? sc[q] : (x == o ? cf[q] : 0.f);
-                }
-                uint2 th, tl;
-                split4(scm, th, tl, spc);
-                tile_store(XS_OFF + wv * 1024, th, tl);
-                publish(TAG_SC, tagv);
-            }
-#pragma unroll
-            for (int jt = 0; jt < 4; ++jt) ST[0][jt] = CK[jt];
-            WKV6_T(ts1);
-            if (grp & 1) {
-                advance(kpart(grp - 1, 0), ST[0], ST[0]);
-                advance(kpart(grp - 1, 1), ST[0], ST[0]);
-            }
-            [[maybe_unused]] unsigned pk_gc = 0;
-#pragma unroll
-            for (int blk = 0; blk < SBLK - 1; ++blk) advance(kpart(grp, blk), ST[blk], ST[blk + 1]);
-            const unsigned pk_da = peek4(TAG_DA);
-            WKV6_T(ts2);
-            f4v ackp[SBLK];
-            float at[SBLK][4], vgs[SBLK];
-            uint2 held_gr[SBLK];
-#pragma unroll
-            for (int blk = SBLK - 1; blk >= 0; --blk) {
-                const char* const rb = rpart(grp, blk);
-                const char* const kb = kpart(grp, blk);
-                b8v gyr[2];
-#pragma unroll
-                for (int s = 0; s < 2; ++s) gyr[s] = ld_b8(rb + R_GY * ARR + x * RSB + (32 * s + 8 * g) * 2);
-                const float vg = *reinterpret_cast<const float*>(rb + ROFF_VG + x * 4) + *reinterpret_cast<const float*>(rb + ROFF_VG + 64 + x * 4);
-                vgs[blk] = vg;
-                if (blk == SBLK - 1) settle4(TAG_DA, grp + 1, pk_da);
-                if constexpr (!SPLIT) { if (blk == 0) pk_gc = peek4(TAG_GC); }
-                const uint4 fab = tile_load(XT_OFF + (2 * blk) * 1024), fba = tile_load(XT_OFF + (2 * blk + 1) * 1024);
-                const s4v dab_hi = __builtin_bit_cast(s4v, make_uint2(fab.x, fab.y)), dab_lo = __builtin_bit_cast(s4v, make_uint2(fab.z, fab.w));
-                const s4v dba_hi = __builtin_bit_cast(s4v, make_uint2(fba.x, fba.y)), dba_lo = __builtin_bit_cast(s4v, make_uint2(fba.z, fba.w));
-                const s4v rhf_w = tr_read(rb + R_RH * ARR + troff + 32 * wv);
-                const s4v rlf_w = tr_read(rb + R_RL * ARR + troff + 32 * wv);
-                const s4v khf = tr_read(kb + K_KH * ARR + troff + 32 * wv);
-                const s4v klf = tr_read(kb + K_KL * ARR + troff + 32 * wv);
-                const float4 e8o = *reinterpret_cast<const float4*>(rb + ROFF_E8 + (16 * wv + 4 * g) * 4);
-                f4v accs = {0.f, 0.f, 0.f, 0.f};
-#pragma unroll
-                for (int s = 0; s < 2; ++s) {
-                    float t0[4], t1[4];
-                    b8v hi, lo;
-#pragma unroll
-                    for (int q = 0; q < 4; ++q) { t0[q] = ST[blk][2 * s][q]; t1[q] = ST[blk][2 * s + 1][q]; }
-                    split8(t0, t1, hi, lo, spc);
-                    accs = mfma32(hi, gyr[s], accs);
-                    accs = mfma32(lo, gyr[s], accs);
-                }
-                f4v accr16 = {0.f, 0.f, 0.f, 0.f};
-                accr16 = mfma16(khf, dba_hi, accr16);
-                accr16 = mfma16(khf, dba_lo, accr16);
-                accr16 = mfma16(klf, dba_hi, accr16);
-                const f4v accr = {fmaf(e8o.x, accs[0], accr16[0]), fmaf(e8o.y, accs[1], accr16[1]),
-                                  fmaf(e8o.z, accs[2], accr16[2]), fmaf(e8o.w, accs[3], accr16[3])};
-                f4v ak = {0.f, 0.f, 0.f, 0.f};
-                ak = mfma16(rhf_w, dab_hi, ak);
-                ak = mfma16(rhf_w, dab_lo, ak);
-                ak = mfma16(rlf_w, dab_hi, ak);
-                ackp[blk] = ak;
-                {
-                    const int ch = 16 * wv + 4 * g;
-                    const float4 fr4 = *reinterpret_cast<const float4*>(rb + ROFF_FR + x * FRS + ch * 4);
-                    const uint2 rr = *reinterpret_cast<const uint2*>(rb + R_R * ARR + x * RSB + ((ch * 2) ^ ((x & 8) << 1)));
-                    const uint2 kk = *reinterpret_cast<const uint2*>(rb + R_K * ARR + x * RSB + ((ch * 2) ^ ((x & 8) << 1)));
-                    const float frv[4] = {fr4.x, fr4.y, fr4.z, fr4.w};
-                    const float rv[4] = {bf_lo(rr.x), bf_hi(rr.x), bf_lo(rr.y), bf_hi(rr.y)};
-                    const float kv[4] = {bf_lo(kk.x), bf_hi(kk.x), bf_lo(kk.y), bf_hi(kk.y)};
-                    float o_gr[4];
-#pragma unroll
-                    for (int q = 0; q < 4; ++q) {
-                        const float dq = frv[q] * accr[q];
-                        o_gr[q] = fmaf(vg * ue[q], kv[q], dq);
-                        gu_acc[q] = fmaf(vg * rv[q], kv[q], gu_acc[q]);
-                        at[blk][q] = rv[q] * dq;
-                    }
-                    held_gr[blk] = emit(0, grp, blk, REV_R, o_gr, old_gr[blk]);
-                }
-            }
-            WKV6_T(ts3);
-#pragma unroll
-            for (int blk = SBLK - 1; blk >= 0; --blk) {
-                fetch_old(1, rs_gk, grp * STG + blk * BLK, REV_K, old_gk[blk]);
-                fetch_old(3, rs_gw, grp * STG + blk * BLK, REV_W, old_gw[blk]);
-            }
-            if (grp > 0 && !(grp & 1)) request_ckpt(grp - 1);
-            if constexpr (CHAIN) {
-                if (nx_chain && grp == 0) {
-                    const rsrc_t rs_nx = make_rsrc(ch.nx_ckpt + ((long)ch.nx_b * a.H + (long)(ch.nx_bh % (unsigned)a.H)) * nslots * (HEAD * HEAD), nslots * 16384u);
-                    const unsigned off = (unsigned)((nxn - 1) >> 1) * 16384u + (unsigned)wv * 4096u + (unsigned)lane * 16u;
-#pragma unroll
-                    for (int jt = 0; jt < 4; ++jt) {
-                        const float4 t = buf_load16f(rs_nx, off + jt * 1024u);
-                        CK[jt] = f4v{t.x, t.y, t.z, t.w};
-                    }
-                }
-            }
-            if constexpr (!SPLIT) {
-                settle4(TAG_GC, grp + 1, pk_gc);
-                gvb[0] = take_gop(0);
-                publish(TAG_GD, tagv);
-            }
-#pragma unroll
-            for (int blk = SBLK - 1; blk >= 0; --blk) put(0, rs_gr, grp, blk, REV_R, held_gr[blk]);
-#pragma unroll
-            for (int blk = SBLK - 1; blk >= 0; --blk) {
-                const char* const rb = rpart(grp, blk);
-                const char* const kb = kpart(grp, blk);
-                f4v acck = {0.f, 0.f, 0.f, 0.f};
-                [[maybe_unused]] f4v Oi[4];
-                [[maybe_unused]] float e8x = 0.f, e16x = 0.f;
-                if constexpr (SPLIT) {
-                    e8x = *reinterpret_cast<const float*>(rb + ROFF_E8 + (16 * wv + x) * 4);
-                    e16x = *reinterpret_cast<const float*>(kb + KOFF_E16 + (16 * wv + x) * 4);
-                    const float e16m8x = *reinterpret_cast<const float*>(kb + KOFF_E16M8 + (16 * wv + x) * 4);
-                    const s4v rhf_w = tr_read(rb + R_RH * ARR + troff + 32 * wv);
-                    const s4v rlf_w = tr_read(rb + R_RL * ARR + troff + 32 * wv);
-#pragma unroll
-                    for (int jt = 0; jt < 4; ++jt) {
-                        const s4v gyf = tr_read(rb + R_GY * ARR + trow + tile_tr(jt));
-                        f4v o = {0.f, 0.f, 0.f, 0.f};
-                        o = mfma32(cat2(gyf, gyf), cat2(rhf_w, rlf_w), o);
-                        Oi[jt] = o;
-                    }
-#pragma unroll
-                    for (int s = 0; s < 2; ++s) {
-                        const b8v vr = ld_b8(kb + K_V * ARR + x * RSB + (32 * s + 8 * g) * 2);
-                        float t0[4], t1[4];
-                        b8v hi, lo;
-#pragma unroll
-                        for (int q = 0; q < 4; ++q) { t0[q] = GI[2 * s][q] * e16m8x; t1[q] = GI[2 * s + 1][q] * e16m8x; }
-                        split8(t0, t1, hi, lo, spc);
-                        acck = mfma32(hi, vr, acck);
-                        acck = mfma32(lo, vr, acck);
-                    }
-                } else {
-                    acck = gvb[blk];
-                }
-                acck += ackp[blk];
-                {
-                    const int ch = 16 * wv + 4 * g;
-                    const float4 fn4 = *reinterpret_cast<const float4*>(x < 15 ? rb + ROFF_FR + (x + 1) * FRS + ch * 4 : kb + KOFF_E16M8 + ch * 4);
-                    const float4 fk4 = make_float4(__builtin_amdgcn_rcpf(fn4.x), __builtin_amdgcn_rcpf(fn4.y), __builtin_amdgcn_rcpf(fn4.z),
-                                                   __builtin_amdgcn_rcpf(fn4.w));
-                    const float4 lw4 = *reinterpret_cast<const float4*>(rb + ROFF_LW + x * FRS + ch * 4);
-                    const uint2 rr = *reinterpret_cast<const uint2*>(rb + R_R * ARR + x * RSB + ((ch * 2) ^ ((x & 8) << 1)));
-                    const uint2 kk = *reinterpret_cast<const uint2*>(rb + R_K * ARR + x * RSB + ((ch * 2) ^ ((x & 8) << 1)));
-                    const float fkv[4] = {fk4.x, fk4.y, fk4.z, fk4.w}, lwv[4] = {lw4.x, lw4.y, lw4.z, lw4.w};
-                    const float rv[4] = {bf_lo(rr.x), bf_hi(rr.x), bf_lo(rr.y), bf_hi(rr.y)};
-                    const float kv[4] = {bf_lo(kk.x), bf_hi(kk.x), bf_lo(kk.y), bf_hi(kk.y)};
-                    const float vg = vgs[blk];
-                    float o_gk[4], o_gw[4], bt[4], dl[4], sfx[4];
-#pragma unroll
-                    for (int q = 0; q < 4; ++q) {
-                        const float dk = fkv[q] * acck[q];
-                        o_gk[q] = fmaf(vg * ue[q], rv[q], dk);
-                        bt[q] = kv[q] * dk;
-                        dl[q] = at[blk][q] - bt[q];
-                        sfx[q] = dl[q];
-                    }
-                    WKV6_DPP_ACC4(sfx, "row_shl:1");
-                    WKV6_DPP_ACC4(sfx, "row_shl:2");
-                    WKV6_DPP_ACC4(sfx, "row_shl:4");
-                    WKV6_DPP_ACC4(sfx, "row_shl:8");
-#pragma unroll
-                    for (int q = 0; q < 4; ++q) {
-                        const float total = dpp_mov<DPP_BCAST0>(sfx[q]);
-                        o_gw[q] = (Rc[q] + (sfx[q] - dl[q]) - bt[q]) * lwv[q];
-                        Rc[q] += total;
-                    }
-                    put(1, rs_gk, grp, blk, REV_K, emit(1, grp, blk, REV_K, o_gk, old_gk[blk]));
-                    put(3, rs_gw, grp, blk, REV_W, emit(3, grp, blk, REV_W, o_gw, old_gw[blk]));
-                }
-                if constexpr (SPLIT) {
-#pragma unroll
-                    for (int jt = 0; jt < 4; ++jt)
-#pragma unroll
-                        for (int q = 0; q < 4; ++q) GI[jt][q] = fmaf(e16x, GI[jt][q], e8x * Oi[jt][q]);
-                }
-            }
-            WKV6_T(ts4);
+        auto stage_barrier = [&]() __attribute__((always_inline)) {
             __syncthreads();
             WKV6_T(ts5);
             WKV6_ACC(0, ts1, ts0); WKV6_ACC(1, ts2, ts1); WKV6_ACC(2, ts3, ts2); WKV6_ACC(3, ts4, ts3); WKV6_ACC(4, ts5, ts4);
+        };
+        if constexpr (!PAIR_WALK) {
+            for (int grp = ngrp - 1; grp >= 0; --grp) {
+                constexpr int PAR = PAR_RUNTIME;
+#include "wkv6_chunk_bwd12k_row_stage.inc"
+                stage_barrier();
+            }
+        } else {
+            auto stage = [&](auto par_c, const int grp) __attribute__((always_inline)) {
+                constexpr int PAR = decltype(par_c)::value;
+#include "wkv6_chunk_bwd12k_row_stage.inc"
+            };
+            int grp = ngrp - 1;
+            if (grp >= 0 && !(grp & 1)) { stage(par_t<PAR_EVEN>{}, grp); stage_barrier(); --grp; }
+            for (; grp >= 1; grp -= 2) {
+                stage(par_t<PAR_ODD>{}, grp); stage_barrier();
+                stage(par_t<PAR_EVEN>{}, grp - 1); stage_barrier();
+            }
         }
         if (a.gu) {
             float s4[4];
 #pragma unroll
             for (int q = 0; q < 4; ++q) s4[q] = row_sum16(gu_acc[q]);
-            const long o = (long)b * a.C + h * HEAD + 16 * wv + 4 * g;
+            int g_gu = g;
+            if constexpr (PAIR_WALK) { int t_ = tid; asm volatile("" : "+v"(t_)); g_gu = (t_ & 63) >> 4; }
+            const long o = (long)b * a.C + h * HEAD + 16 * wv + 4 * g_gu;
             if (x == 0) {
                 if (a.part_f32) io4<float>::store(reinterpret_cast<float*>(a.gu) + o, s4);
                 else io4<bf16_t>::store(reinterpret_cast<bf16_t*>(a.gu) + o, s4);
@@ -881,177 +672,33 @@
         }
         __syncthreads();
         if constexpr (!SPLIT) { if (ngrp > 0) scale_split(kpart(ngrp - 1, SBLK - 1), nh, nl); }
-        for (int grp = ngrp - 1; grp >= 0; --grp) {
-            int tagv = grp + 1;
-            for (int i_ = 0; i_ < wv; ++i_) __builtin_amdgcn_s_sleep(2);
-            asm volatile("" : "+v"(tagv));
-            WKV6_T(ts0);
-
-            s4v gyT_w[SBLK], sc_hi[SBLK], sc_lo[SBLK];
-            f4v accp[SBLK];
-            b8v gh[SBLK][2], gl[SBLK][2];
-            [[maybe_unused]] f4v Og[SBLK][4];
-            if constexpr (!SPLIT)
-#pragma unroll
-            for (int blk = SBLK - 1; blk >= 0; --blk) {
-                const char* const rb = rpart(grp, blk);
-                const char* const kb = kpart(grp, blk);
-                if (blk == SBLK - 1) {
-#pragma unroll
-                    for (int s = 0; s < 2; ++s) { gh[blk][s] = nh[s]; gl[blk][s] = nl[s]; }
-                    if (grp == ngrp - 1) {
-                        gop_write(gh[blk], gl[blk]);
-                        publish(TAG_GA, tagv);
-                    }
-                    if constexpr (CHAIN) {
-                        const bool g_nx = nx_chain && grp == 0, v_nx = nx_chain && grp <= 1;
-                        load_gy(g_nx ? nx : cur, g_nx ? lp_vg_nx : lp_vg, g_nx ? nxn - 1 : grp - 1);
-                        load_v(v_nx ? nx : cur, v_nx ? lp_vg_nx : lp_vg, v_nx ? (grp == 1 ? nxn - 1 : nxn - 2) : grp - 2);
-                    } else {
-                        if (grp > 0) load_gy(cur, lp_vg, grp - 1);
-                        if (grp > 1) load_v(cur, lp_vg, grp - 2);
-                    }
-                } else {
-                    scale_split(kb, gh[blk], gl[blk]);
-                    await4(TAG_GB, grp + 1);
-                    gop_write(gh[blk], gl[blk]);
-                    publish(TAG_GC, tagv);
-                }
-                const s4v gyT = tr_read(rb + R_GY * ARR + troff + 32 * wv);
-#pragma unroll
-                for (int it = 0; it < 4; ++it) {
-                    const s4v rhf = tr_read(rb + R_RH * ARR + trow + tile_tr(it));
-                    const s4v rlf = tr_read(rb + R_RL * ARR + trow + tile_tr(it));
-                    f4v o = {0.f, 0.f, 0.f, 0.f};
-                    o = mfma32(cat2(rhf, rlf), cat2(gyT, gyT), o);
-                    const float4 d16 = *reinterpret_cast<const float4*>(kb + KOFF_E16 + (tile_ch(it) + 8 * g) * 4);
-                    const float4 d8 = *reinterpret_cast<const float4*>(rb + ROFF_E8 + (tile_ch(it) + 8 * g) * 4);
-                    GJ[it][0] = fmaf(d16.x, GJ[it][0], d8.x * o[0]);
-                    GJ[it][1] = fmaf(d16.y, GJ[it][1], d8.y * o[1]);
-                    GJ[it][2] = fmaf(d16.z, GJ[it][2], d8.z * o[2]);
-                    GJ[it][3] = fmaf(d16.w, GJ[it][3], d8.w * o[3]);
-                }
-            }
-            float old_gv[SBLK][4] = {};
-#pragma unroll
-            for (int blk = SBLK - 1; blk >= 0; --blk) fetch_old(2, rs_gv, grp * STG + blk * BLK, REV_V, old_gv[blk]);
-            if (SPLIT && wv < SBLK) {
-                const char* const rb = rpart(grp, wv);
-                const char* const kb = kpart(grp, wv);
-                f4v sc = {0.f, 0.f, 0.f, 0.f};
-#pragma unroll
-                for (int s = 0; s < 2; ++s) {
-                    const int off = x * RSB + (32 * s + 8 * g) * 2;
-                    const b8v rh = ld_b8(rb + R_RH * ARR + off), rl = ld_b8(rb + R_RL * ARR + off);
-                    const b8v kh = ld_b8(kb + K_KH * ARR + off), kl = ld_b8(kb + K_KL * ARR + off);
-                    sc = mfma32(rh, kh, sc);
-                    sc = mfma32(rh, kl, sc);
-                    sc = mfma32(rl, kh, sc);
-                }
-                const float4 cfa = *reinterpret_cast<const float4*>(rb + ROFF_COEF + 16 * g);
-                const float4 cfb = *reinterpret_cast<const float4*>(rb + ROFF_COEF + 64 + 16 * g);
-                const float cf[4] = {cfa.x + cfb.x, cfa.y + cfb.y, cfa.z + cfb.z, cfa.w + cfb.w};
-                float scm[4];
-#pragma unroll
-                for (int q = 0; q < 4; ++q) {
-                    const int o = 4 * g + q;
-                    scm[q] = x < o ? sc[q] : (x == o ? cf[q] : 0.f);
-                }
-                uint2 th, tl;
-                split4(scm, th, tl, spc);
-                tile_store(XS_OFF + wv * 1024, th, tl);
-                publish(TAG_SC, tagv);
-            }
-#pragma unroll
-            for (int blk = 0; blk < SBLK; ++blk) gyT_w[blk] = tr_read(rpart(grp, blk) + R_GY * ARR + troff + 32 * wv);
-#pragma unroll
-            for (int blk = 0; blk < SBLK; ++blk) {
-                if (blk == 0) await2(TAG_SC, grp + 1);
-                const uint4 f = tile_load(XS_OFF + blk * 1024);
-                sc_hi[blk] = __builtin_bit_cast(s4v, make_uint2(f.x, f.y));
-                sc_lo[blk] = __builtin_bit_cast(s4v, make_uint2(f.z, f.w));
-            }
-#pragma unroll
-            for (int blk = 0; blk < SBLK; ++blk) {
-                f4v acc = {0.f, 0.f, 0.f, 0.f};
-                acc = mfma32(cat2(gyT_w[blk], gyT_w[blk]), cat2(sc_hi[blk], sc_lo[blk]), acc);
-                accp[blk] = acc;
-                if constexpr (SPLIT) {
-                    const char* const rb = rpart(grp, blk);
-#pragma unroll
-                    for (int it = 0; it < 4; ++it) {
-                        const s4v rhf = tr_read(rb + R_RH * ARR + trow + tile_tr(it));
-                        const s4v rlf = tr_read(rb + R_RL * ARR + trow + tile_tr(it));
-                        f4v o = {0.f, 0.f, 0.f, 0.f};
-                        o = mfma32(cat2(rhf, rlf), cat2(gyT_w[blk], gyT_w[blk]), o);
-                        Og[blk][it] = o;
-                    }
-                }
-            }
-            WKV6_T(ts1);
-            uint2 held_gv[SBLK];
-#pragma unroll
-            for (int blk = SBLK - 1; blk >= 0; --blk) {
-                const char* const kb = kpart(grp, blk);
-                f4v acc = {0.f, 0.f, 0.f, 0.f};
-#pragma unroll
-                for (int s = 0; s < 2; ++s) {
-                    const int off = x * RSB + (32 * s + 8 * g) * 2;
-                    const b8v kh = ld_b8(kb + K_KH * ARR + off), kl = ld_b8(kb + K_KL * ARR + off);
-                    if constexpr (SPLIT) {
-                        float t0[4], t1[4];
-                        const float4 m0 = *reinterpret_cast<const float4*>(kb + KOFF_E16M8 + (32 * s + 8 * g) * 4);
-                        const float4 m1 = *reinterpret_cast<const float4*>(kb + KOFF_E16M8 + (32 * s + 8 * g + 4) * 4);
-                        t0[0] = GJ[2 * s][0] * m0.x; t0[1] = GJ[2 * s][1] * m0.y; t0[2] = GJ[2 * s][2] * m0.z; t0[3] = GJ[2 * s][3] * m0.w;
-                        t1[0] = GJ[2 * s + 1][0] * m1.x; t1[1] = GJ[2 * s + 1][1] * m1.y;
-                        t1[2] = GJ[2 * s + 1][2] * m1.z; t1[3] = GJ[2 * s + 1][3] * m1.w;
-                        split8(t0, t1, gh[blk][s], gl[blk][s], spc);
-                    }
-                    acc = mfma32(gh[blk][s], kh, acc);
-                    acc = mfma32(gh[blk][s], kl, acc);
-                    acc = mfma32(gl[blk][s], kh, acc);
-                }
-                acc += accp[blk];
-                {
-                    float o[4] = {acc[0], acc[1], acc[2], acc[3]};
-                    held_gv[blk] = emit(2, grp, blk, REV_V, o, old_gv[blk]);
-                }
-                if constexpr (SPLIT) {
-                    const char* const rb = rpart(grp, blk);
-#pragma unroll
-                    for (int it = 0; it < 4; ++it) {
-                        const float4 d16 = *reinterpret_cast<const float4*>(kb + KOFF_E16 + (tile_ch(it) + 8 * g) * 4);
-                        const float4 d8 = *reinterpret_cast<const float4*>(rb + ROFF_E8 + (tile_ch(it) + 8 * g) * 4);
-                        GJ[it][0] = fmaf(d16.x, GJ[it][0], d8.x * Og[blk][it][0]);
-                        GJ[it][1] = fmaf(d16.y, GJ[it][1], d8.y * Og[blk][it][1]);
-                        GJ[it][2] = fmaf(d16.z, GJ[it][2], d8.z * Og[blk][it][2]);
-                        GJ[it][3] = fmaf(d16.w, GJ[it][3], d8.w * Og[blk][it][3]);
-                    }
-                }
-            }
-#pragma unroll
-            for (int blk = SBLK - 1; blk >= 0; --blk) put(2, rs_gv, grp, blk, REV_V, held_gv[blk]);
-            if constexpr (!SPLIT) {
-                if (grp > 0) {
-                    scale_split(kpart(grp - 1, SBLK - 1), nh, nl);
-                    await4(TAG_GD, grp + 1);
-                    gop_write(nh, nl);
-                    publish(TAG_GA, tagv - 1);
-                }
-            }
-            if constexpr (!SPLIT) {
-                if (grp > 0) copy_gy(rpart(grp - 1, 0));
-                else if (CHAIN && nx_chain) copy_gy(rpart_nx(0, 0));
-                if (grp > 1) copy_v(kpart(grp - 2, 0));
-                else if (CHAIN && nx_chain) copy_v(grp == 1 ? kpart_nx(0, 0) : kpart_nx(1, 0));
-            }
-            WKV6_T(ts2);
+        auto stage_barrier = [&]() __attribute__((always_inline)) {
             __syncthreads();
             WKV6_T(ts3);
             WKV6_ACC(0, ts1, ts0); WKV6_ACC(1, ts2, ts1); WKV6_ACC(2, ts3, ts2);
+        };
+        if constexpr (!PAIR_WALK) {
+            for (int grp = ngrp - 1; grp >= 0; --grp) {
+                constexpr int PAR = PAR_RUNTIME;
+#include "wkv6_chunk_bwd12k_col_stage.inc"
+                stage_barrier();
+            }
+        } else {
+            auto stage = [&](auto par_c, const int grp) __attribute__((always_inline)) {
+                constexpr int PAR = decltype(par_c)::value;
+#include "wkv6_chunk_bwd12k_col_stage.inc"
+            };
+            int grp = ngrp - 1;
+            if (grp >= 0 && !(grp & 1)) { stage(par_t<PAR_EVEN>{}, grp); stage_barrier(); --grp; }
+            for (; grp >= 1; grp -= 2) {
+                stage(par_t<PAR_ODD>{}, grp); stage_barrier();
+                stage(par_t<PAR_EVEN>{}, grp - 1); stage_barrier();
+            }
         }
         if (a.gs) {
-            const long so_ = ((long)b * a.H + h) * HEAD * HEAD + (long)(16 * wv + x) * HEAD + 8 * g;
+            int x_gs = x, g_gs = g;
+            if constexpr (PAIR_WALK) { int t_ = tid; asm volatile("" : "+v"(t_)); x_gs = t_ & 15; g_gs = (t_ & 63) >> 4; }
+            const long so_ = ((long)b * a.H + h) * HEAD * HEAD + (long)(16 * wv + x_gs) * HEAD + 8 * g_gs;
 #pragma unroll
             for (int it = 0; it < 4; ++it) {
                 const float t4[4] = {GJ[it][0], GJ[it][1], GJ[it][2], GJ[it][3]};
diff --git a/rwkv_lm_ext_amd/csrc/wkv6_chunk_bwd12k_col_stage.inc b/rwkv_lm_ext_amd/csrc/wkv6_chunk_bwd12k_col_stage.inc
--- /dev/null
+++ b/rwkv_lm_ext_amd/csrc/wkv6_chunk_bwd12k_col_stage.inc
@@ -0,0 +1,165 @@
+            if constexpr (PAR != PAR_RUNTIME && !R1_HOIST) asm volatile("" : "+s"(rbuf1));
+            int tagv = grp + 1;
+            for (int i_ = 0; i_ < wv; ++i_) __builtin_amdgcn_s_sleep(2);
+            asm volatile("" : "+v"(tagv));
+            WKV6_T(ts0);
+
+            s4v gyT_w[SBLK], sc_hi[SBLK], sc_lo[SBLK];
+            f4v accp[SBLK];
+            b8v gh[SBLK][2], gl[SBLK][2];
+            [[maybe_unused]] f4v Og[SBLK][4];
+            if constexpr (!SPLIT)
+#pragma unroll
+            for (int blk = SBLK - 1; blk >= 0; --blk) {
+                const char* const rb = rpart_p(par_t<PAR>{}, grp, blk);
+                const char* const kb = kpart(grp, blk);
+                if (blk == SBLK - 1) {
+#pragma unroll
+                    for (int s = 0; s < 2; ++s) { gh[blk][s] = nh[s]; gl[blk][s] = nl[s]; }
+                    if (grp == ngrp - 1) {
+                        gop_write(gh[blk], gl[blk]);
+                        publish(TAG_GA, tagv);
+                    }
+                    if constexpr (CHAIN) {
+                        const bool g_nx = nx_chain && grp == 0, v_nx = nx_chain && grp <= 1;
+                        load_gy(g_nx ? nx : cur, g_nx ? lp_vg_nx : lp_vg, g_nx ? nxn - 1 : grp - 1);
+                        load_v(v_nx ? nx : cur, v_nx ? lp_vg_nx : lp_vg, v_nx ? (grp == 1 ? nxn - 1 : nxn - 2) : grp - 2);
+                    } else {
+                        if (PAR == PAR_ODD || grp > 0) load_gy(cur, lp_vg, grp - 1);
+                        if (grp > 1) load_v(cur, lp_vg, grp - 2);
+                    }
+                } else {
+                    scale_split(kb, gh[blk], gl[blk]);
+                    await4(TAG_GB, grp + 1);
+                    gop_write(gh[blk], gl[blk]);
+                    publish(TAG_GC, tagv);
+                }
+                const s4v gyT = tr_read(rb + R_GY * ARR + troff + 32 * wv);
+#pragma unroll
+                for (int it = 0; it < 4; ++it) {
+                    const s4v rhf = tr_read(rb + R_RH * ARR + trow + tile_tr(it));
+                    const s4v rlf = tr_read(rb + R_RL * ARR + trow + tile_tr(it));
+                    f4v o = {0.f, 0.f, 0.f, 0.f};
+                    o = mfma32(cat2(rhf, rlf), cat2(gyT, gyT), o);
+                    const float4 d16 = *reinterpret_cast<const float4*>(kb + KOFF_E16 + (tile_ch(it) + 8 * g) * 4);
+                    const float4 d8 = *reinterpret_cast<const float4*>(rb + ROFF_E8 + (tile_ch(it) + 8 * g) * 4);
+                    GJ[it][0] = fmaf(d16.x, GJ[it][0], d8.x * o[0]);
+                    GJ[it][1] = fmaf(d16.y, GJ[it][1], d8.y * o[1]);
+                    GJ[it][2] = fmaf(d16.z, GJ[it][2], d8.z * o[2]);
+                    GJ[it][3] = fmaf(d16.w, GJ[it][3], d8.w * o[3]);
+                }
+            }
+            float old_gv[SBLK][4] = {};
+#pragma unroll
+            for (int blk = SBLK - 1; blk >= 0; --blk) fetch_old(2, rs_gv, grp * STG + blk * BLK, REV_V, old_gv[blk]);
+            if (SPLIT && wv < SBLK) {
+                const char* const rb = rpart_p(par_t<PAR>{}, grp, wv);
+                const char* const kb = kpart(grp, wv);
+                f4v sc = {0.f, 0.f, 0.f, 0.f};
+#pragma unroll
+                for (int s = 0; s < 2; ++s) {
+                    const int off = x * RSB + (32 * s + 8 * g) * 2;
+                    const b8v rh = ld_b8(rb + R_RH * ARR + off), rl = ld_b8(rb + R_RL * ARR + off);
+                    const b8v kh = ld_b8(kb + K_KH * ARR + off), kl = ld_b8(kb + K_KL * ARR + off);
+                    sc = mfma32(rh, kh, sc);
+                    sc = mfma32(rh, kl, sc);
+                    sc = mfma32(rl, kh, sc);
+                }
+                const float4 cfa = *reinterpret_cast<const float4*>(rb + ROFF_COEF + 16 * g);
+                const float4 cfb = *reinterpret_cast<const float4*>(rb + ROFF_COEF + 64 + 16 * g);
+                const float cf[4] = {cfa.x + cfb.x, cfa.y + cfb.y, cfa.z + cfb.z, cfa.w + cfb.w};
+                float scm[4];
+#pragma unroll
+                for (int q = 0; q < 4; ++q) {
+                    const int o = 4 * g + q;
+                    scm[q] = x < o ? sc[q] : (x == o ? cf[q] : 0.f);
+                }
+                uint2 th, tl;
+                split4(scm, th, tl, spc);
+                tile_store(XS_OFF + wv * 1024, th, tl);
+                publish(TAG_SC, tagv);
+            }
+#pragma unroll
+            for (int blk = 0; blk < SBLK; ++blk) gyT_w[blk] = tr_read(rpart_p(par_t<PAR>{}, grp, blk) + R_GY * ARR + troff + 32 * wv);
+#pragma unroll
+            for (int blk = 0; blk < SBLK; ++blk) {
+                if (blk == 0) await2(TAG_SC, grp + 1);
+                const uint4 f = tile_load(XS_OFF + blk * 1024);
+                sc_hi[blk] = __builtin_bit_cast(s4v, make_uint2(f.x, f.y));
+                sc_lo[blk] = __builtin_bit_cast(s4v, make_uint2(f.z, f.w));
+            }
+#pragma unroll
+            for (int blk = 0; blk < SBLK; ++blk) {
+                f4v acc = {0.f, 0.f, 0.f, 0.f};
+                acc = mfma32(cat2(gyT_w[blk], gyT_w[blk]), cat2(sc_hi[blk], sc_lo[blk]), acc);
+                accp[blk] = acc;
+                if constexpr (SPLIT) {
+                    const char* const rb = rpart_p(par_t<PAR>{}, grp, blk);
+#pragma unroll
+                    for (int it = 0; it < 4; ++it) {
+                        const s4v rhf = tr_read(rb + R_RH * ARR + trow + tile_tr(it));
+                        const s4v rlf = tr_read(rb + R_RL * ARR + trow + tile_tr(it));
+                        f4v o = {0.f, 0.f, 0.f, 0.f};
+                        o = mfma32(cat2(rhf, rlf), cat2(gyT_w[blk], gyT_w[blk]), o);
+                        Og[blk][it] = o;
+                    }
+                }
+            }
+            WKV6_T(ts1);
+            uint2 held_gv[SBLK];
+#pragma unroll
+            for (int blk = SBLK - 1; blk >= 0; --blk) {
+                const char* const kb = kpart(grp, blk);
+                f4v acc = {0.f, 0.f, 0.f, 0.f};
+#pragma unroll
+                for (int s = 0; s < 2; ++s) {
+                    const int off = x * RSB + (32 * s + 8 * g) * 2;
+                    const b8v kh = ld_b8(kb + K_KH * ARR + off), kl = ld_b8(kb + K_KL * ARR + off);
+                    if constexpr (SPLIT) {
+                        float t0[4], t1[4];
+                        const float4 m0 = *reinterpret_cast<const float4*>(kb + KOFF_E16M8 + (32 * s + 8 * g) * 4);
+                        const float4 m1 = *reinterpret_cast<const float4*>(kb + KOFF_E16M8 + (32 * s + 8 * g + 4) * 4);
+                        t0[0] = GJ[2 * s][0] * m0.x; t0[1] = GJ[2 * s][1] * m0.y; t0[2] = GJ[2 * s][2] * m0.z; t0[3] = GJ[2 * s][3] * m0.w;
+                        t1[0] = GJ[2 * s + 1][0] * m1.x; t1[1] = GJ[2 * s + 1][1] * m1.y;
+                        t1[2] = GJ[2 * s + 1][2] * m1.z; t1[3] = GJ[2 * s + 1][3] * m1.w;
+                        split8(t0, t1, gh[blk][s], gl[blk][s], spc);
+                    }
+                    acc = mfma32(gh[blk][s], kh, acc);
+                    acc = mfma32(gh[blk][s], kl, acc);
+                    acc = mfma32(gl[blk][s], kh, acc);
+                }
+                acc += accp[blk];
+                {
+                    float o[4] = {acc[0], acc[1], acc[2], acc[3]};
+                    held_gv[blk] = emit(2, grp, blk, REV_V, o, old_gv[blk]);
+                }
+                if constexpr (SPLIT) {
+                    const char* const rb = rpart_p(par_t<PAR>{}, grp, blk);
+#pragma unroll
+                    for (int it = 0; it < 4; ++it) {
+                        const float4 d16 = *reinterpret_cast<const float4*>(kb + KOFF_E16 + (tile_ch(it) + 8 * g) * 4);
+                        const float4 d8 = *reinterpret_cast<const float4*>(rb + ROFF_E8 + (tile_ch(it) + 8 * g) * 4);
+                        GJ[it][0] = fmaf(d16.x, GJ[it][0], d8.x * Og[blk][it][0]);
+                        GJ[it][1] = fmaf(d16.y, GJ[it][1], d8.y * Og[blk][it][1]);
+                        GJ[it][2] = fmaf(d16.z, GJ[it][2], d8.z * Og[blk][it][2]);
+                        GJ[it][3] = fmaf(d16.w, GJ[it][3], d8.w * Og[blk][it][3]);
+                    }
+                }
+            }
+#pragma unroll
+            for (int blk = SBLK - 1; blk >= 0; --blk) put(2, rs_gv, grp, blk, REV_V, held_gv[blk]);
+            if constexpr (!SPLIT) {
+                if (PAR == PAR_ODD || grp > 0) {
+                    scale_split(kpart(grp - 1, SBLK - 1), nh, nl);
+                    await4(TAG_GD, grp + 1);
+                    gop_write(nh, nl);
+                    publish(TAG_GA, tagv - 1);
+                }
+            }
+            if constexpr (!SPLIT) {
+                if (PAR == PAR_ODD || grp > 0) copy_gy(rpart_p(par_other_t<PAR>{}, grp - 1, 0));
+                else if (CHAIN && nx_chain) copy_gy(rpart_nx(0, 0));
+                if (grp > 1) copy_v(kpart(grp - 2, 0));
+                else if (CHAIN && nx_chain) copy_v(grp == 1 ? kpart_nx(0, 0) : kpart_nx(1, 0));
+            }
+            WKV6_T(ts2);
diff --git a/rwkv_lm_ext_amd/csrc/wkv6_chunk_bwd12k_row_stage.inc b/rwkv_lm_ext_amd/csrc/wkv6_chunk_bwd12k_row_stage.inc
--- /dev/null
+++ b/rwkv_lm_ext_amd/csrc/wkv6_chunk_bwd12k_row_stage.inc
@@ -0,0 +1,273 @@
+            if constexpr (PAR != PAR_RUNTIME && !R1_HOIST) asm volatile("" : "+s"(rbuf1));
+            int tagv = grp + 1;
+            asm volatile("" : "+v"(tagv));
+            WKV6_T(ts0);
+            f4v gvb[SBLK];
+            auto take_gop = [&](int blk) {
+                int base_ = GOP_OFF + (8 * g + (x >> 2)) * GRS + (16 * wv + 4 * (x & 3)) * 2;
+                asm volatile("" : "+v"(base_));
+                typedef short s8v __attribute__((ext_vector_type(8)));
+                const char* const kb = kpart(grp, blk);
+                f4v acc = {0.f, 0.f, 0.f, 0.f};
+#pragma unroll
+                for (int s = 0; s < 2; ++s) {
+                    const char* const ph = smem + base_ + 32 * s * GRS;
+                    const s8v h8 = __builtin_shufflevector(tr_read(ph), tr_read(ph + 4 * GRS), 0, 1, 2, 3, 4, 5, 6, 7);
+                    const s8v l8 = __builtin_shufflevector(tr_read(ph + HEAD * GRS), tr_read(ph + HEAD * GRS + 4 * GRS), 0, 1, 2, 3, 4, 5, 6, 7);
+                    const b8v vr = ld_b8(kb + K_V * ARR + x * RSB + (32 * s + 8 * g) * 2);
+                    acc = mfma32(__builtin_bit_cast(b8v, h8), vr, acc);
+                    acc = mfma32(__builtin_bit_cast(b8v, l8), vr, acc);
+                }
+                return acc;
+            };
+            if constexpr (!SPLIT) {
+                if (grp == ngrp - 1) await4(TAG_GA, grp + 1);
+                gvb[1] = take_gop(1);
+                publish(TAG_GB, tagv);
+            }
+            float old_gr[SBLK][4] = {}, old_gk[SBLK][4] = {}, old_gw[SBLK][4] = {};
+#pragma unroll
+            for (int blk = SBLK - 1; blk >= 0; --blk) fetch_old(0, rs_gr, grp * STG + blk * BLK, REV_R, old_gr[blk]);
+            if (wv >= 2) {
+                const int tb = wv - 2;
+                const char* const rb = rpart_p(par_t<PAR>{}, grp, tb);
+                const char* const kb = kpart(grp, tb);
+                f4v dA_ab = {0.f, 0.f, 0.f, 0.f}, dA_ba = {0.f, 0.f, 0.f, 0.f};
+#pragma unroll
+                for (int s = 0; s < 2; ++s) {
+                    const int off = x * RSB + (32 * s + 8 * g) * 2;
+                    const b8v gy_ = ld_b8(rb + R_GY * ARR + off), vr = ld_b8(kb + K_V * ARR + off);
+                    dA_ab = mfma32(gy_, vr, dA_ab);
+                    dA_ba = mfma32(vr, gy_, dA_ba);
+                }
+                float dab[4], dba[4];
+#pragma unroll
+                for (int q = 0; q < 4; ++q) {
+                    const int o = 4 * g + q;
+                    dab[q] = x < o ? dA_ab[q] : 0.f;
+                    dba[q] = o < x ? dA_ba[q] : 0.f;
+                }
+                uint2 th, tl;
+                split4(dab, th, tl, spc);
+                tile_store(XT_OFF + (2 * tb) * 1024, th, tl);
+                publish_at(tag_tb, TAG_DA, 0, tagv);
+                split4(dba, th, tl, spc);
+                tile_store(XT_OFF + (2 * tb + 1) * 1024, th, tl);
+                publish_at(tag_tb, TAG_DA, 4, tagv);
+            } else if constexpr (!SPLIT) {
+                const char* const rb = rpart_p(par_t<PAR>{}, grp, wv);
+                const char* const kb = kpart(grp, wv);
+                f4v sc = {0.f, 0.f, 0.f, 0.f};
+#pragma unroll
+                for (int s = 0; s < 2; ++s) {
+                    const int off = x * RSB + (32 * s + 8 * g) * 2;
+                    const b8v rh = ld_b8(rb + R_RH * ARR + off), rl = ld_b8(rb + R_RL * ARR + off);
+                    const b8v kh = ld_b8(kb + K_KH * ARR + off), kl = ld_b8(kb + K_KL * ARR + off);
+                    sc = mfma32(rh, kh, sc);
+                    sc = mfma32(rh, kl, sc);
+                    sc = mfma32(rl, kh, sc);
+                }
+                const float4 cfa = *reinterpret_cast<const float4*>(rb + ROFF_COEF + 16 * g);
+                const float4 cfb = *reinterpret_cast<const float4*>(rb + ROFF_COEF + 64 + 16 * g);
+                const float cf[4] = {cfa.x + cfb.x, cfa.y + cfb.y, cfa.z + cfb.z, cfa.w + cfb.w};
+                float scm[4];
+#pragma unroll
+                for (int q = 0; q < 4; ++q) {
+                    const int o = 4 * g + q;
+                    scm[q] = x < o ? sc[q] : (x == o ? cf[q] : 0.f);
+                }
+                uint2 th, tl;
+                split4(scm, th, tl, spc);
+                tile_store(XS_OFF + wv * 1024, th, tl);
+                publish(TAG_SC, tagv);
+            }
+            if constexpr (PAR == PAR_RUNTIME) {
+#pragma unroll
+                for (int jt = 0; jt < 4; ++jt) ST[0][jt] = CK[jt];
+            }
+            WKV6_T(ts1);
+            if constexpr (PAR == PAR_RUNTIME) {
+                if (grp & 1) {
+                    advance(kpart(grp - 1, 0), ST[0], ST[0]);
+                    advance(kpart(grp - 1, 1), ST[0], ST[0]);
+                }
+            } else if constexpr (PAR == PAR_ODD) {
+                advance(kpart(grp - 1, 0), CK, ST[0]);
+                advance(kpart(grp - 1, 1), ST[0], ST[0]);
+            }
+            const f4v (&S0)[4] = [&]() -> const f4v (&)[4] { if constexpr (PAR == PAR_EVEN) return CK; else return ST[0]; }();
+            [[maybe_unused]] unsigned pk_gc = 0;
+            static_assert(SBLK == 2, "block 0 enters with S0, block 1 with ST[1]");
+            advance(kpart(grp, 0), S0, ST[1]);
+            const unsigned pk_da = peek4(TAG_DA);
+            WKV6_T(ts2);
+            f4v ackp[SBLK];
+            float at[SBLK][4], vgs[SBLK];
+            uint2 held_gr[SBLK];
+#pragma unroll
+            for (int blk = SBLK - 1; blk >= 0; --blk) {
+                const char* const rb = rpart_p(par_t<PAR>{}, grp, blk);
+                const char* const kb = kpart(grp, blk);
+                b8v gyr[2];
+#pragma unroll
+                for (int s = 0; s < 2; ++s) gyr[s] = ld_b8(rb + R_GY * ARR + x * RSB + (32 * s + 8 * g) * 2);
+                const float vg = *reinterpret_cast<const float*>(rb + ROFF_VG + x * 4) + *reinterpret_cast<const float*>(rb + ROFF_VG + 64 + x * 4);
+                vgs[blk] = vg;
+                if (blk == SBLK - 1) settle4(TAG_DA, grp + 1, pk_da);
+                if constexpr (!SPLIT) { if (blk == 0) pk_gc = peek4(TAG_GC); }
+                const uint4 fab = tile_load(XT_OFF + (2 * blk) * 1024), fba = tile_load(XT_OFF + (2 * blk + 1) * 1024);
+                const s4v dab_hi = __builtin_bit_cast(s4v, make_uint2(fab.x, fab.y)), dab_lo = __builtin_bit_cast(s4v, make_uint2(fab.z, fab.w));
+                const s4v dba_hi = __builtin_bit_cast(s4v, make_uint2(fba.x, fba.y)), dba_lo = __builtin_bit_cast(s4v, make_uint2(fba.z, fba.w));
+                const s4v rhf_w = tr_read(rb + R_RH * ARR + troff + 32 * wv);
+                const s4v rlf_w = tr_read(rb + R_RL * ARR + troff + 32 * wv);
+                const s4v khf = tr_read(kb + K_KH * ARR + troff + 32 * wv);
+                const s4v klf = tr_read(kb + K_KL * ARR + troff + 32 * wv);
+                const float4 e8o = *reinterpret_cast<const float4*>(rb + ROFF_E8 + (16 * wv + 4 * g) * 4);
+                f4v accs = {0.f, 0.f, 0.f, 0.f};
+                const f4v (&Sb)[4] = blk ? ST[blk] : S0;
+#pragma unroll
+                for (int s = 0; s < 2; ++s) {
+                    float t0[4], t1[4];
+                    b8v hi, lo;
+#pragma unroll
+                    for (int q = 0; q < 4; ++q) { t0[q] = Sb[2 * s][q]; t1[q] = Sb[2 * s + 1][q]; }
+                    split8(t0, t1, hi, lo, spc);
+                    accs = mfma32(hi, gyr[s], accs);
+                    accs = mfma32(lo, gyr[s], accs);
+                }
+                f4v accr16 = {0.f, 0.f, 0.f, 0.f};
+                accr16 = mfma16(khf, dba_hi, accr16);
+                accr16 = mfma16(khf, dba_lo, accr16);
+                accr16 = mfma16(klf, dba_hi, accr16);
+                const f4v accr = {fmaf(e8o.x, accs[0], accr16[0]), fmaf(e8o.y, accs[1], accr16[1]),
+                                  fmaf(e8o.z, accs[2], accr16[2]), fmaf(e8o.w, accs[3], accr16[3])};
+                f4v ak = {0.f, 0.f, 0.f, 0.f};
+                ak = mfma16(rhf_w, dab_hi, ak);
+                ak = mfma16(rhf_w, dab_lo, ak);
+                ak = mfma16(rlf_w, dab_hi, ak);
+                ackp[blk] = ak;
+                {
+                    const int ch = 16 * wv + 4 * g;
+                    const float4 fr4 = *reinterpret_cast<const float4*>(rb + ROFF_FR + x * FRS + ch * 4);
+                    const uint2 rr = *reinterpret_cast<const uint2*>(rb + R_R * ARR + x * RSB + ((ch * 2) ^ ((x & 8) << 1)));
+                    const uint2 kk = *reinterpret_cast<const uint2*>(rb + R_K * ARR + x * RSB + ((ch * 2) ^ ((x & 8) << 1)));
+                    const float frv[4] = {fr4.x, fr4.y, fr4.z, fr4.w};
+                    const float rv[4] = {bf_lo(rr.x), bf_hi(rr.x), bf_lo(rr.y), bf_hi(rr.y)};
+                    const float kv[4] = {bf_lo(kk.x), bf_hi(kk.x), bf_lo(kk.y), bf_hi(kk.y)};
+                    float o_gr[4];
+#pragma unroll
+                    for (int q = 0; q < 4; ++q) {
+                        const float dq = frv[q] * accr[q];
+                        o_gr[q] = fmaf(vg * ue[q], kv[q], dq);
+                        gu_acc[q] = fmaf(vg * rv[q], kv[q], gu_acc[q]);
+                        at[blk][q] = rv[q] * dq;
+                    }
+                    held_gr[blk] = emit(0, grp, blk, REV_R, o_gr, old_gr[blk]);
+                }
+            }
+            WKV6_T(ts3);
+#pragma unroll
+            for (int blk = SBLK - 1; blk >= 0; --blk) {
+                fetch_old(1, rs_gk, grp * STG + blk * BLK, REV_K, old_gk[blk]);
+                fetch_old(3, rs_gw, grp * STG + blk * BLK, REV_W, old_gw[blk]);
+            }
+            if constexpr (PAR == PAR_RUNTIME) { if (grp > 0 && !(grp & 1)) request_ckpt(grp - 1); }
+            else if constexpr (PAR == PAR_EVEN) request_ckpt(grp > 0 ? grp - 1 : 2 * (int)nslots);
+            if constexpr (CHAIN) {
+                if (nx_chain && grp == 0) {
+                    const rsrc_t rs_nx = make_rsrc(ch.nx_ckpt + ((long)ch.nx_b * a.H + (long)(ch.nx_bh % (unsigned)a.H)) * nslots * (HEAD * HEAD), nslots * 16384u);
+                    const unsigned off = (unsigned)((nxn - 1) >> 1) * 16384u + (unsigned)wv * 4096u + (unsigned)lane * 16u;
+#pragma unroll
+                    for (int jt = 0; jt < 4; ++jt) {
+                        const float4 t = buf_load16f(rs_nx, off + jt * 1024u);
+                        CK[jt] = f4v{t.x, t.y, t.z, t.w};
+                    }
+                }
+            }
+            if constexpr (!SPLIT) {
+                settle4(TAG_GC, grp + 1, pk_gc);
+                gvb[0] = take_gop(0);
+                publish(TAG_GD, tagv);
+            }
+#pragma unroll
+            for (int blk = SBLK - 1; blk >= 0; --blk) put(0, rs_gr, grp, blk, REV_R, held_gr[blk]);
+            [[maybe_unused]] int rsel = PAR == PAR_ODD ? RBUF_BYTES : 0;
+            if constexpr (PAR != PAR_RUNTIME) asm volatile("" : "+s"(rsel));
+#pragma unroll
+            for (int blk = SBLK - 1; blk >= 0; --blk) {
+                const char* const rb = rpart_p(par_t<PAR>{}, grp, blk);
+                const char* const rb_sel = [&]() { if constexpr (PAR == PAR_RUNTIME) return rb; else return smem + rsel + blk * RBLK_BYTES; }();
+                const char* const kb = kpart(grp, blk);
+                f4v acck = {0.f, 0.f, 0.f, 0.f};
+                [[maybe_unused]] f4v Oi[4];
+                [[maybe_unused]] float e8x = 0.f, e16x = 0.f;
+                if constexpr (SPLIT) {
+                    e8x = *reinterpret_cast<const float*>(rb + ROFF_E8 + (16 * wv + x) * 4);
+                    e16x = *reinterpret_cast<const float*>(kb + KOFF_E16 + (16 * wv + x) * 4);
+                    const float e16m8x = *reinterpret_cast<const float*>(kb + KOFF_E16M8 + (16 * wv + x) * 4);
+                    const s4v rhf_w = tr_read(rb + R_RH * ARR + troff + 32 * wv);
+                    const s4v rlf_w = tr_read(rb + R_RL * ARR + troff + 32 * wv);
+#pragma unroll
+                    for (int jt = 0; jt < 4; ++jt) {
+                        const s4v gyf = tr_read(rb + R_GY * ARR + trow + tile_tr(jt));
+                        f4v o = {0.f, 0.f, 0.f, 0.f};
+                        o = mfma32(cat2(gyf, gyf), cat2(rhf_w, rlf_w), o);
+                        Oi[jt] = o;
+                    }
+#pragma unroll
+                    for (int s = 0; s < 2; ++s) {
+                        const b8v vr = ld_b8(kb + K_V * ARR + x * RSB + (32 * s + 8 * g) * 2);
+                        float t0[4], t1[4];
+                        b8v hi, lo;
+#pragma unroll
+                        for (int q = 0; q < 4; ++q) { t0[q] = GI[2 * s][q] * e16m8x; t1[q] = GI[2 * s + 1][q] * e16m8x; }
+                        split8(t0, t1, hi, lo, spc);
+                        acck = mfma32(hi, vr, acck);
+                        acck = mfma32(lo, vr, acck);
+                    }
+                } else {
+                    acck = gvb[blk];
+                }
+                acck += ackp[blk];
+                {
+                    const int ch = 16 * wv + 4 * g;
+                    const float4 fn4 = *reinterpret_cast<const float4*>(x < 15 ? rb_sel + ROFF_FR + (x + 1) * FRS + ch * 4 : kb + KOFF_E16M8 + ch * 4);
+                    const float4 fk4 = make_float4(__builtin_amdgcn_rcpf(fn4.x), __builtin_amdgcn_rcpf(fn4.y), __builtin_amdgcn_rcpf(fn4.z),
+                                                   __builtin_amdgcn_rcpf(fn4.w));
+                    const float4 lw4 = *reinterpret_cast<const float4*>(rb + ROFF_LW + x * FRS + ch * 4);
+                    const uint2 rr = *reinterpret_cast<const uint2*>(rb + R_R * ARR + x * RSB + ((ch * 2) ^ ((x & 8) << 1)));
+                    const uint2 kk = *reinterpret_cast<const uint2*>(rb + R_K * ARR + x * RSB + ((ch * 2) ^ ((x & 8) << 1)));
+                    const float fkv[4] = {fk4.x, fk4.y, fk4.z, fk4.w}, lwv[4] = {lw4.x, lw4.y, lw4.z, lw4.w};
+                    const float rv[4] = {bf_lo(rr.x), bf_hi(rr.x), bf_lo(rr.y), bf_hi(rr.y)};
+                    const float kv[4] = {bf_lo(kk.x), bf_hi(kk.x), bf_lo(kk.y), bf_hi(kk.y)};
+                    const float vg = vgs[blk];
+                    float o_gk[4], o_gw[4], bt[4], dl[4], sfx[4];
+#pragma unroll
+                    for (int q = 0; q < 4; ++q) {
+                        const float dk = fkv[q] * acck[q];
+                        o_gk[q] = fmaf(vg * ue[q], rv[q], dk);
+                        bt[q] = kv[q] * dk;
+                        dl[q] = at[blk][q] - bt[q];
+                        sfx[q] = dl[q];
+                    }
+                    WKV6_DPP_ACC4(sfx, "row_shl:1");
+                    WKV6_DPP_ACC4(sfx, "row_shl:2");
+                    WKV6_DPP_ACC4(sfx, "row_shl:4");
+                    WKV6_DPP_ACC4(sfx, "row_shl:8");
+#pragma unroll
+                    for (int q = 0; q < 4; ++q) {
+                        const float total = dpp_mov<DPP_BCAST0>(sfx[q]);
+                        o_gw[q] = (Rc[q] + (sfx[q] - dl[q]) - bt[q]) * lwv[q];
+                        Rc[q] += total;
+                    }
+                    put(1, rs_gk, grp, blk, REV_K, emit(1, grp, blk, REV_K, o_gk, old_gk[blk]));
+                    put(3, rs_gw, grp, blk, REV_W, emit(3, grp, blk, REV_W, o_gw, old_gw[blk]));
+                }
+                if constexpr (SPLIT) {
+#pragma unroll
+                    for (int jt = 0; jt < 4; ++jt)
+#pragma unroll
+                        for (int q = 0; q < 4; ++q) GI[jt][q] = fmaf(e16x, GI[jt][q], e8x * Oi[jt][q]);
+                }
+            }
+            WKV6_T(ts4);
```

After: 58.06 million, median of 6. About the same (+1.0%).
